# reginald-mclean/mtrl

Hardware: AMD Instinct MI355X
Metric: SAC gradient-steps/sec, MT50 width-2048 batch=128/task, 1/2/4/8 MI355X (higher is better)
Workload: dtype fp32 (2xfp16 split, per-tensor power-of-two scaled, 3 fp16 MFMA products, fp32-accurate); 1 GPU; MT50 MTMHSAC-v2 width=2048 (experiments/width_scaling/mt50_mtmhsac_v2_2048.py); num_tasks=50, width=2048, batch_per_task=128, global_batch=6400, parallelism=single, precision=split2h, exec=pipelined

## Files before the change

### include/mtsac_debug.h

```cpp
#ifndef MTSAC_DEBUG_H_
#define MTSAC_DEBUG_H_

#include <stdint.h>

#ifdef __cplusplus
extern "C" {
#endif

int mtsac_debug_gemm(int precision, int kind, int epi, int batch, int M, int N, int K, const float* A, int lda, int a_shared,
                     const float* B, int ldb, float* C, int ldc, const float* bias, const float* mask, int ldm,
                     float* db);

int mtsac_debug_gemm_bench(int precision, int kind, int epi, int batch, int M, int N, int K, int iters,
                           double* ms_per_launch);

int mtsac_debug_gemm_x3p(int epi, int M, int N, int K, const float* A, int a_kmajor, const float* B, int b_kmajor,
                         float* C, const float* bias, const float* mask, float* Csum);
int mtsac_debug_gemm_x3p_bench(int epi, int batch, int M, int N, int K, int iters, double* ms_per_launch);
int mtsac_debug_x3p_geo(int geo);

int mtsac_debug_gemm_x3f(int epi, int batch, int M, int N, int K, const float* A, const float* B, float* C,
                         const float* bias, const float* mask, float* Csum);
int mtsac_debug_gemm_x3f_ragged(int flags, int B, int N, int K, const float* A, const float* W, const float* mask,
                                const unsigned char* active, void* dense_out, void* rag_out, int* rows_out, int* info);
int mtsac_debug_gemm_fwd_bench(int which, int epi, int batch, int M, int N, int K, int iters, double* ms_per_launch);
int mtsac_debug_x3s_ti(int M, int N, int batch);
int mtsac_debug_drq_groups(int fwd, int bwd);
int mtsac_debug_drq_mfma(int mask);
int mtsac_debug_drq_legacy(int mask);
int mtsac_debug_drq_wgrad_blocks(int cap);
int mtsac_debug_drq_conv_bench(int kind, int B, int H, int W, int ci, int co, int iters, double* us_per_launch);

int mtsac_debug_drq_conv(int kind, int flags, int B, int B1, int H, int W, int ci, int co, const float* x,
                         const float* w, const float* bias, const float* w2, const float* bias2, const float* aux,
                         const float* aux2, float* out, float* out2);
int mtsac_debug_drq_conv_path(int kind, int B, int H, int W, int ci, int co, int* out);
int mtsac_debug_drq_maxpool(int B, int H, int W, int C, const float* in, float* out, unsigned char* arg,
                            const float* dout, float* din);
int mtsac_debug_drq_c51(int B, int A, int Z, int ldh, const float* hc_s, const float* hc_n, const float* hc_t,
                        const float* hb_on, const float* hb_tg, const float* rew, const float* done, const int* act,
                        float gamma_n, float vmin, float vmax, float* m, int* a_next, float* q, float* dh,
                        float* loss_b, float* logit_b);

struct mtsac_engine;
int mtsac_debug_set_pipeline(struct mtsac_engine* engine, int32_t on);

int mtsac_debug_lane_mode(struct mtsac_engine* engine);
int mtsac_debug_check_guards(struct mtsac_engine* engine);
int mtsac_debug_snapshot(struct mtsac_engine* engine, int32_t on);
int mtsac_debug_read(struct mtsac_engine* engine, int32_t id, float* dst, int64_t count);
int mtsac_debug_head_selfcheck(struct mtsac_engine* engine);
int mtsac_debug_set_bfrag(int32_t mode);
int mtsac_debug_set_actor_dense(int32_t mode);
int mtsac_debug_actor_compact(struct mtsac_engine* engine);
int mtsac_debug_bfrag(struct mtsac_engine* engine);
int mtsac_debug_force_one_stream(struct mtsac_engine* engine, int32_t on);
int mtsac_debug_set_collective_model(struct mtsac_engine* engine, int32_t nranks, double bus_gbps, int32_t flags);

struct mtsac_engine;
int mtsac_debug_timed_launch(struct mtsac_engine* engine, int32_t i, int32_t* dims, double* ms);

#ifdef __cplusplus
}
#endif
#endif
```

### mtrl_amd/_lib.py

```python

from __future__ import annotations

import ctypes
import os
import pathlib

_HERE = pathlib.Path(__file__).resolve().parent
LIB_PATH = pathlib.Path(os.environ.get("MTSAC_LIB", _HERE / "libmtsac.so"))

NUM_LOGS = 10
FP32, FP32_SPLIT3, BF16, FP32_SPLIT2H = 0, 1, 2, 3
PRECISIONS = {"fp32": FP32, "split3": FP32_SPLIT3, "bf16": BF16, "split2h": FP32_SPLIT2H}
LOG_KEYS = (
    "losses/qf_values",
    "losses/qf_loss",
    "metrics/critic_grad_magnitude",
    "metrics/critic_params_norm",
    "losses/actor_loss",
    "metrics/actor_grad_magnitude",
    "metrics/actor_params_norm",
    "metrics/explore_loss",
    "losses/alpha_loss",
    "alpha",
)
# ... 65 lines not shown
    "mtsac_last_error": (ctypes.c_char_p, []),
    "mtsac_abi_version": (ctypes.c_int, []),
    "mtsac_build_stamp": (ctypes.c_char_p, []),
    "mtsac_default_config": (None, [ctypes.POINTER(Config), I32]),
    "mtsac_create": (ctypes.c_int, [ctypes.POINTER(Config), ctypes.c_int, ctypes.POINTER(P)]),
    "mtsac_destroy": (None, [P]),
    "mtsac_param_count": (I64, [P, ctypes.c_int]),
    "mtsac_set_params": (ctypes.c_int, [P, ctypes.c_int, P, I64]),
    "mtsac_get_params": (ctypes.c_int, [P, ctypes.c_int, P, I64]),
    "mtsac_set_adam_count": (ctypes.c_int, [P, ctypes.c_int, I32]),
    "mtsac_get_adam_count": (ctypes.c_int, [P, ctypes.c_int, PI32]),
    "mtsac_buffer_add": (ctypes.c_int, [P, P, P, P, P, P]),
    "mtsac_buffer_add_stream": (ctypes.c_int, [P, P, P, P, P, P, P]),
    "mtsac_buffer_write": (ctypes.c_int, [P, I64, I64, P, P, P, P, P]),
    "mtsac_buffer_read": (ctypes.c_int, [P, I64, I64, P, P, P, P, P]),
    "mtsac_buffer_fill_synthetic": (ctypes.c_int, [P, U64]),
    "mtsac_buffer_set_state": (ctypes.c_int, [P, I64, I32]),
    "mtsac_buffer_get_state": (ctypes.c_int, [P, PI64, PI32]),
    "mtsac_buffer_set_reward_stats": (ctypes.c_int, [P, PD, PD]),
    "mtsac_buffer_get_reward_stats": (ctypes.c_int, [P, PD, PD]),
    "mtsac_rng_set": (ctypes.c_int, [P, U64, U64, U64, U64, I32, U32]),
    "mtsac_rng_get": (ctypes.c_int, [P, PU64, PU64, PU64, PU64, PI32, PU32]),
    "mtsac_sample": (ctypes.c_int, [P, P, P, P, P, P, P]),
    "mtsac_update": (ctypes.c_int, [P, ctypes.POINTER(Batch), P, P]),
    "mtsac_update_many": (ctypes.c_int, [P, I32]),
    "mtsac_get_logs": (ctypes.c_int, [P, P]),
    "mtsac_enable_graph": (ctypes.c_int, [P, I32]),
    "mtsac_synchronize": (ctypes.c_int, [P]),
    "mtsac_eval_action": (ctypes.c_int, [P, P, I32, P]),
    "mtsac_sample_action": (ctypes.c_int, [P, P, I32, P, P]),
    "mtsac_comm_unique_id_size": (ctypes.c_int, []),
    "mtsac_comm_get_unique_id": (ctypes.c_int, [P]),
    "mtsac_comm_init": (ctypes.c_int, [P, P, I32, I32]),
    "mtsac_comm_init_timeout": (ctypes.c_int, [P, P, I32, I32, ctypes.c_double]),
    "mtsac_comm_nranks": (ctypes.c_int, [P, P]),
    "mtsac_get_noise_state": (ctypes.c_int, [P, P, P]),
    "mtsac_set_noise_state": (ctypes.c_int, [P, ctypes.c_uint64, ctypes.c_uint64]),
    "mtsac_set_allreduce_hook": (ctypes.c_int, [P, ctypes.c_void_p, P]),
    "mtsac_set_collective_hook": (ctypes.c_int, [P, ctypes.c_void_p, P, ctypes.c_int32, ctypes.c_int32]),
    "mtsac_set_sharded_optimizer": (ctypes.c_int, [P, ctypes.c_int32]),
    "mtsac_memcpy": (ctypes.c_int, [P, P, I64]),
    "mtsac_set_timing": (ctypes.c_int, [P, I32]),
    "mtsac_get_timing": (ctypes.c_int, [P, I32, PD, PI32, PD]),
    "mtsac_get_timing_kernel": (ctypes.c_int, [P, I32, P, I32]),
    "mtsac_task_gradients": (ctypes.c_int, [P, ctypes.POINTER(Batch), P, P]),
    "mtsac_task_gradient_size": (I64, [P, ctypes.c_int]),
    "mtsac_get_task_gradients": (ctypes.c_int, [P, ctypes.c_int, P, I64]),
    "mtsac_set_task_gradients": (ctypes.c_int, [P, ctypes.c_int, P, I64]),
    "mtsac_task_gradient_select": (ctypes.c_int, [P, ctypes.c_int, P, P]),
    "mtsac_task_gradient_stats": (ctypes.c_int, [P, ctypes.c_int, P, ctypes.c_float, ctypes.c_float, P, P, P, P]),
    "mtsac_set_pcgrad": (ctypes.c_int, [P, I32, I32]),
    "mtsac_pcgrad_set_order": (ctypes.c_int, [P, P, P]),
    "mtsac_pcgrad_get_order": (ctypes.c_int, [P, P, P]),
    "mtsac_get_pcgrad_logs": (ctypes.c_int, [P, P]),
    "mtsac_task_gram": (ctypes.c_int, [P, ctypes.c_int, P]),
    "mtsac_task_pcgrad_solve": (ctypes.c_int, [P, ctypes.c_int, P, I32, P, P]),
    "mtsac_task_combine": (ctypes.c_int, [P, ctypes.c_int, P, P]),
    "mtsac_debug_gemm_bench": (ctypes.c_int, [ctypes.c_int] * 8 + [PD]),
    "mtsac_debug_gemm_x3p": (ctypes.c_int, [ctypes.c_int] * 4 + [P, ctypes.c_int, P, ctypes.c_int, P, P, P, P]),
    "mtsac_debug_gemm_x3p_bench": (ctypes.c_int, [ctypes.c_int] * 6 + [PD]),
    "mtsac_debug_x3p_geo": (ctypes.c_int, [ctypes.c_int]),
    "mtsac_debug_gemm_x3f": (ctypes.c_int, [ctypes.c_int] * 5 + [P] * 6),
    "mtsac_debug_gemm_x3f_ragged": (ctypes.c_int, [ctypes.c_int] * 4 + [P] * 8),
    "mtsac_debug_gemm_fwd_bench": (ctypes.c_int, [ctypes.c_int] * 7 + [PD]),
    "mtsac_debug_x3s_ti": (ctypes.c_int, [ctypes.c_int] * 3),
    "mtsac_debug_drq_groups": (ctypes.c_int, [ctypes.c_int] * 2),
    "mtsac_debug_drq_mfma": (ctypes.c_int, [ctypes.c_int]),
    "mtsac_debug_drq_legacy": (ctypes.c_int, [ctypes.c_int]),
    "mtsac_debug_drq_wgrad_blocks": (ctypes.c_int, [ctypes.c_int]),
    "mtsac_debug_drq_conv_bench": (ctypes.c_int, [ctypes.c_int] * 7 + [ctypes.POINTER(ctypes.c_double)]),
    "mtsac_debug_drq_conv": (ctypes.c_int, [ctypes.c_int] * 8 + [P] * 9),
    "mtsac_debug_drq_conv_path": (ctypes.c_int, [ctypes.c_int] * 6 + [P]),
    "mtsac_debug_drq_maxpool": (ctypes.c_int, [ctypes.c_int] * 4 + [P] * 5),
    "mtsac_debug_drq_c51": (ctypes.c_int, [ctypes.c_int] * 4 + [P] * 8 + [ctypes.c_float] * 3 + [P] * 6),
    "mtsac_debug_set_pipeline": (ctypes.c_int, [P, I32]),
    "mtsac_debug_lane_mode": (ctypes.c_int, [P]),
    "mtsac_debug_check_guards": (ctypes.c_int, [P]),
    "mtsac_debug_snapshot": (ctypes.c_int, [P, ctypes.c_int32]),
    "mtsac_debug_read": (ctypes.c_int, [P, ctypes.c_int32, P, ctypes.c_int64]),
    "mtsac_debug_head_selfcheck": (ctypes.c_int, [P]),
    "mtsac_debug_set_bfrag": (ctypes.c_int, [ctypes.c_int32]),
    "mtsac_debug_set_actor_dense": (ctypes.c_int, [ctypes.c_int32]),
    "mtsac_debug_actor_compact": (ctypes.c_int, [P]),
    "mtsac_debug_bfrag": (ctypes.c_int, [P]),
    "mtsac_debug_force_one_stream": (ctypes.c_int, [P, ctypes.c_int32]),
    "mtsac_debug_set_collective_model": (ctypes.c_int, [P, ctypes.c_int32, ctypes.c_double, ctypes.c_int32]),
    "mtsac_debug_timed_launch": (ctypes.c_int, [P, I32, PI32, PD]),
    "mtsac_debug_gemm": (
        ctypes.c_int,
        [ctypes.c_int] * 7 + [P, ctypes.c_int, ctypes.c_int, P, ctypes.c_int, P, ctypes.c_int, P, P, ctypes.c_int, P],
    ),
}


class DrqConfig(ctypes.Structure):
    _fields_ = [(n, ctypes.c_int32) for n in ("num_tasks", "n_actions", "n_atoms", "in_ch", "hw", "scale",
                                              "embed_dim", "n_hidden", "batch", "nstep")] + \
               [(n, ctypes.c_float) for n in ("gamma", "v_min", "v_max", "tau", "lr", "b1", "b2", "eps",
                                              "weight_decay", "ln_eps")] + \
               [("capacity", ctypes.c_int64), ("normalize_rewards", ctypes.c_int32), ("buffer_kind", ctypes.c_int32)]


class DrqBatch(ctypes.Structure):
    _fields_ = [(n, ctypes.c_void_p) for n in ("obs", "actions", "next_obs", "dones", "rewards", "task_ids",
                                               "crop_obs", "noise_obs", "crop_next", "noise_next")]


DRQ_PARAMS, DRQ_TARGET, DRQ_ADAM_MU, DRQ_ADAM_NU, DRQ_GRAD = 0, 1, 2, 3, 4
DRQ_NUM_LOGS = 4
DRQ_LOG_KEYS = ("losses/online_logits", "metrics/critic_grad_magnitude", "metrics/critic_params_norm",
                "losses/critic_loss")
SIGNATURES.update({
    "drq_last_error": (ctypes.c_char_p, []),
    "drq_create": (ctypes.c_int, [ctypes.POINTER(DrqConfig), ctypes.c_int, ctypes.POINTER(P)]),
    "drq_destroy": (None, [P]),
    "drq_num_params": (I64, [P]),
    "drq_set_params": (ctypes.c_int, [P, ctypes.c_int, P, I64]),
    "drq_get_params": (ctypes.c_int, [P, ctypes.c_int, P, I64]),
    "drq_set_step": (ctypes.c_int, [P, ctypes.c_int]),
    "drq_get_step": (ctypes.c_int, [P, P]),
    "drq_update": (ctypes.c_int, [P, ctypes.POINTER(DrqBatch)]),
    "drq_update_resident": (ctypes.c_int, [P, ctypes.c_int]),
    "drq_get_logs": (ctypes.c_int, [P, P]),
    "drq_q_values": (ctypes.c_int, [P, P, P, P, P, ctypes.c_int, P]),
    "drq_buffer_add": (ctypes.c_int, [P, P, P, P, P, P, P]),
    "drq_buffer_state": (ctypes.c_int, [P, PI64, PI32]),
    "drq_rng_set": (ctypes.c_int, [P, U64, U64, U64, U64, ctypes.c_int, U32]),
    "drq_sample": (ctypes.c_int, [P]),
    "drq_sample_update": (ctypes.c_int, [P, ctypes.c_int]),
    "drq_sample_rows": (ctypes.c_int, [P, P, P]),
    "drq_sample_rows_update": (ctypes.c_int, [P, P, P, ctypes.c_int]),
    "drq_rng_get": (ctypes.c_int, [P, P]),
    "drq_seed_augment": (ctypes.c_int, [P, ctypes.c_uint64]),
    "drq_task_gradient": (ctypes.c_int, [P, ctypes.POINTER(DrqBatch), ctypes.c_int, ctypes.c_int]),
    "drq_get_task_gradient": (ctypes.c_int, [P, ctypes.c_int, P, I64]),
    "drq_project_task_gradients": (ctypes.c_int, [P, ctypes.c_int, ctypes.c_int, I64, ctypes.c_int, P]),
    "drq_set_timing": (ctypes.c_int, [P, ctypes.c_int]),
    "drq_timing": (ctypes.c_int, [P, P, P, P]),
    "drq_read_batch": (ctypes.c_int, [P, P, P, P, P, P, P, P]),
    "drq_synchronize": (ctypes.c_int, [P]),
})

def source_stamp() -> str | None:
    import hashlib

    csrc = pathlib.Path(__file__).resolve().parent / "csrc"
    if not csrc.is_dir():
        return None
    rel = [f.name for pat in ("*.hip", "*.cpp", "*.h") for f in csrc.glob(pat)]
    rel += ["../../include/" + f.name for f in (csrc / ".." / ".." / "include").glob("*.h")]
    h = hashlib.sha256()
    for r in sorted(rel):
        h.update((csrc / r).read_bytes())
    return h.hexdigest()[:16]


ALLREDUCE_FN = ctypes.CFUNCTYPE(ctypes.c_int, ctypes.c_void_p, ctypes.c_void_p, ctypes.c_int64)
COLLECTIVE_FN = ctypes.CFUNCTYPE(ctypes.c_int, ctypes.c_void_p, ctypes.c_int32, ctypes.c_void_p, ctypes.c_int64)

_lib = None


def load(path: str | os.PathLike | None = None) -> ctypes.CDLL:
    global _lib
    if _lib is not None and path is None:
        return _lib
# ... 35 lines not shown
```

### mtrl_amd/csrc/debug.cpp

```cpp
#include <hip/hip_runtime.h>

#include <algorithm>
#include <cmath>
#include <cstdio>
#include <cstring>
#include <string>
#include <vector>

#include "../../include/mtsac.h"
#include "../../include/mtsac_debug.h"
#include "drq_kernels.h"
#include "kernels.h"

using namespace mtsac;

namespace {

long long up32(long long x) { return (x + 31) / 32 * 32; }

__global__ void fill_rand_f32(float* p, long long n, unsigned seed) {
  long long i = (long long)blockIdx.x * blockDim.x + threadIdx.x;
  if (i >= n) return;
  unsigned x = (unsigned)i * 2654435761u ^ seed;
  x ^= x >> 13;
// ... 434 lines not shown
  };
  std::vector<PlaneRec> hrec(5);
  std::memset(hrec.data(), 0, sizeof(PlaneRec) * hrec.size());
  const float ma = amax(Az.data(), nA), mw = amax(W, nW), mm = amax(mask, nC);
  hrec[0].e = pexp(ma); hrec[0].amax[0] = ma;
  hrec[1].e = pexp(mw); hrec[1].amax[0] = mw;
  hrec[2].e = pexp(mm); hrec[2].amax[0] = mm;
  hrec[3].e = hrec[4].e = 0x7fffffff;
  for (int i = 0; i < PLANE_REC_PARTS; ++i) hrec[3].amax[i] = hrec[4].amax[i] = 1e30f;
  PlaneRec* rec = gd.in(hrec.data(), hrec.size());
  const long long Kp = (K + 63) / 64 * 64;
  __bf16* Azp = gd.mem.get<__bf16>((size_t)3 * B * Kp * E);
  __bf16* Acp = gd.mem.get<__bf16>((size_t)3 * B * Kp * E);
  __bf16* Wp = gd.mem.get<__bf16>((size_t)3 * N * Kp * E);
  __bf16* Mp = gd.mem.get<__bf16>(3 * nC);
  const size_t out_bytes = pout ? nC * 2 * sizeof(__bf16) : nC * sizeof(float);
  unsigned char* dden = gd.out<unsigned char>(out_bytes, "dense out");
  unsigned char* drag = gd.out<unsigned char>(out_bytes, "ragged out");
  if (!gd.ok || !dAc || !rec || !Azp || !Acp || !Wp || !Mp) return -12;
  for (int z = 0; z < E; ++z) {
    SplitParams sp{};
    sp.ldx = K; sp.rows = B; sp.cols = K; sp.ldo = Kp; sp.po = (long long)B * Kp; sp.out_rows = B; sp.out_cols = (int)Kp;
    sp.e2h = &rec[0].e;
    sp.x = dAz + (size_t)z * B * K; sp.out = Azp + (size_t)z * 3 * B * Kp;
    split_planes(sp, false, 1, nullptr);
    sp.x = dAc + (size_t)z * B * K; sp.out = Acp + (size_t)z * 3 * B * Kp;
    split_planes(sp, false, 1, nullptr);
    sp.x = dW + (size_t)z * N * K; sp.rows = N; sp.out = Wp + (size_t)z * 3 * N * Kp; sp.po = (long long)N * Kp;
    sp.out_rows = N; sp.e2h = &rec[1].e; sp.frag = bfrag ? 1 : 0;
    split_planes(sp, false, 1, nullptr);
    sp.frag = 0;
    sp.x = dmask + (size_t)z * B * N; sp.ldx = N; sp.rows = B; sp.cols = N;
    sp.out = Mp + (size_t)z * 3 * B * N; sp.ldo = N; sp.po = (long long)B * N; sp.out_rows = B; sp.out_cols = N;
    sp.e2h = &rec[2].e;
    split_planes(sp, false, 1, nullptr);
  }
  SplitGemmParams g{};
  g.np = 2;
  g.lda = Kp; g.pA = (long long)B * Kp; g.sA = 3 * g.pA;
  g.B = Wp; g.ldb = Kp; g.pB = (long long)N * Kp; g.sB = 3 * g.pB;
  g.b_frag = bfrag ? 1 : 0;
  g.mask16 = Mp; g.ldm = N; g.sMask = 3ll * B * N; g.pMask = (long long)B * N;
  g.M = B; g.N = N; g.K = (int)Kp;
  g.ra = rec + 0; g.na = 1;
  g.rb = rec + 1; g.nb = 1;
  g.kmul = (float)K;
  int nparts[2] = {0, 0};
  auto outs = [&](unsigned char* o, PlaneRec* rc, int* np_) {
    g.C = nullptr; g.Cp = nullptr; g.rc = nullptr;
    if (pout) {
      g.Cp = reinterpret_cast<__bf16*>(o); g.ldcp = N; g.pC = (long long)B * N; g.sCp = 2 * g.pC;
      g.rc = rc;
    } else {
      g.C = reinterpret_cast<float*>(o); g.ldc = N; g.sC = (long long)B * N;
    }
    g.nparts = np_;
  };
  g.A = Azp;
  outs(dden, rec + 3, &nparts[0]);
  gemm_x3f(g, EPI_RELU_MASK, E, nullptr);
  if (int rc = sync_rc("dense gemm_x3f")) return rc;
  g.A = Acp;
  outs(drag, rec + 4, &nparts[1]);
  g.rag_n = d_n; g.rag_rows = d_rows; g.rag_ld = B;
  gemm_x3f_ragged(g, nullptr);
  if (int rc = sync_rc("gemm_x3f_ragged")) return rc;
  if (int rc = gd.check()) return rc;
  if (!gd.back(reinterpret_cast<unsigned char*>(dense_out), dden, out_bytes) ||
      !gd.back(reinterpret_cast<unsigned char*>(rag_out), drag, out_bytes) ||
      !gd.back(hrec.data(), rec, hrec.size()))
    return -5;
  std::copy(hrows.begin(), hrows.end(), rows_out);
  for (int k = 0; k < 2; ++k) {
    float m = 0.f;
    for (int i = 0; i < nparts[k] && i < PLANE_REC_PARTS; ++i) m = std::max(m, hrec[3 + k].amax[i]);
    info[k] = hrec[3 + k].e;
    std::memcpy(&info[2 + k], &m, sizeof(float));
  }
  info[4] = hn[0];
  info[5] = hn[1];
  return 0;
}

int mtsac_debug_gemm_fwd_bench(int which, int epi, int batch, int M, int N, int K, int iters, double* ms_per_launch) {
  const int outs = (epi >> 8) & 3;
  const int np = ((epi >> 10) & 1) ? 1 : 3;
  const bool autosplit = (epi >> 11) & 1;
  const bool fin = (epi >> 12) & 1;
  const bool h2 = (epi >> 13) & 1;
  const bool bfrag = (epi >> 14) & 1;
  epi &= 255;
  if (M < 1 || N < 1 || K < 1 || batch < 1 || iters < 1 || !ms_per_launch) return -22;
  DevBuf d;
  const long long Kp = (K + 63) / 64 * 64;
  PlaneRec* rec = d.get<PlaneRec>(3);
  if (!rec) return -12;
  float* fa = d.get<float>((size_t)M * Kp);
  float* fb = d.get<float>((size_t)N * Kp);
  float* C = d.get<float>((size_t)M * N * batch);
  float* bias = d.get<float>((size_t)N * batch);
  __bf16* Cp = d.get<__bf16>((size_t)3 * M * N * batch);
  if (!fa || !fb || !C || !bias || !Cp) return -12;
  hipLaunchKernelGGL(fill_rand_f32, dim3((unsigned)(((long long)M * Kp + 255) / 256)), dim3(256), 0, nullptr, fa,
                     (long long)M * Kp, 3u);
  hipLaunchKernelGGL(fill_rand_f32, dim3((unsigned)(((long long)N * Kp + 255) / 256)), dim3(256), 0, nullptr, fb,
                     (long long)N * Kp, 5u);
  const bool bk = which == 0;
  long long lda, pa, ldb, pb;
  plane_geom(M, (int)Kp, false, lda, pa);
  plane_geom(N, (int)Kp, bk, ldb, pb);
  __bf16* Ap = d.get<__bf16>((size_t)3 * pa * batch);
  __bf16* Bp = d.get<__bf16>((size_t)3 * pb * batch);
  if (!Ap || !Bp) return -12;
  for (int z = 0; z < batch; ++z) {
    split_into(fa, M, (int)Kp, false, Ap + 3 * pa * z, h2 ? &rec[0].e : nullptr);
    split_into(fb, N, (int)Kp, bk, Bp + 3 * pb * z, h2 ? &rec[1].e : nullptr, bfrag && !bk);
  }
  SplitGemmParams g{};
  if (h2) {
    g.ra = rec; g.rb = rec + 1; g.rc = rec + 2;
    g.kmul = (float)K;
    g.pMask = (long long)M * N;
  }
  g.A = Ap; g.lda = lda; g.pA = pa; g.sA = 3 * pa;
  g.B = Bp; g.ldb = ldb; g.pB = pb; g.sB = 3 * pb; g.b_kmajor = bk;
  g.b_frag = bfrag && !bk ? 1 : 0;
  g.C = C; g.ldc = N; g.sC = (long long)M * N;
  g.bias = bias; g.sBias = N;
  g.mask = C; g.ldm = N; g.sMask = (long long)M * N;
  g.Cp = Cp; g.ldcp = N; g.pC = (long long)M * N; g.sCp = 3 * g.pC;
  if (outs == 1) g.C = nullptr;
  if (outs == 2) g.Cp = nullptr;
  g.M = M; g.N = N; g.K = (int)Kp;
  g.splits = 1;
  g.np = h2 ? 2 : np;
  if (autosplit) {
    const long long wsf = std::max(gemm_x3f_ws_floats(M, N, (int)Kp, batch), gemm_x3p_ws_floats(M, N, (int)Kp, batch, false));
    g.ws = d.get<float>((size_t)std::max(wsf, 1LL));
    if (!g.ws) return -12;
    g.splits = -1;
    if (fin) {
      g.cnt = d.get<int>((size_t)GEMM_X3F_CNT);
      if (!g.cnt) return -12;
    }
  }
  if (which >= 1 && !gemm_x3f_ok(g, epi, batch)) return -95;
  if (which < 0 && !gemm_x3s_ok(g, epi, batch)) return -95;
  auto run = [&]() {
    if (which == -1) gemm_x3s(g, epi, batch, nullptr);
    else if (which < -1) gemm_x3s_ablate(g, -1 - which, batch, nullptr);
    else if (which >= 2) gemm_x3f_ablate(g, which - 2, batch, nullptr);
    else if (which == 1) gemm_x3f(g, epi, batch, nullptr);
    else gemm_x3p(g, epi, batch, nullptr);
  };
  run();
  hipEvent_t e0, e1;
  if (hipEventCreate(&e0) != hipSuccess || hipEventCreate(&e1) != hipSuccess) return -5;
  (void)hipEventRecord(e0, nullptr);
  for (int i = 0; i < iters; ++i) run();
  (void)hipEventRecord(e1, nullptr);
  if (hipEventSynchronize(e1) != hipSuccess) return -5;
  float ms = 0.f;
  (void)hipEventElapsedTime(&ms, e0, e1);
  *ms_per_launch = ms / iters;
  (void)hipEventDestroy(e0);
  (void)hipEventDestroy(e1);
// ... 170 lines not shown
```

### mtrl_amd/csrc/engine.cpp

```cpp
#include <hip/hip_runtime.h>
#include <rccl/rccl.h>

#include <algorithm>
#include <chrono>
#include <cmath>
#include <cstdio>
#include <cstring>
#include <mutex>
#include <string>
#include <thread>
#include <vector>

#include "../../include/mtsac.h"
#include "../../include/mtsac_debug.h"
#include "kernels.h"

using namespace mtsac;

namespace {

thread_local std::string g_last_error;
int g_bfrag_mode = -1;
int g_actor_dense_mode = -1;

int fail(int code, const std::string& msg) {
  g_last_error = msg;
  return code;
}

}
namespace mtsac {
void set_last_error(const char* msg) { g_last_error = msg; }
}
namespace {

#define HIP_TRY(expr)                                                                      \
  do {                                                                                     \
    hipError_t _e = (expr);                                                                \
    if (_e != hipSuccess)                                                                  \
      return fail(-5, std::string(#expr) + ": " + hipGetErrorString(_e));                  \
  } while (0)

constexpr int MAXD = 8;
constexpr long long ALIGN = 64;
constexpr int EXTRA = 128;
constexpr int PART = 1024;

long long align_up(long long x, long long a) { return (x + a - 1) / a * a; }

struct Net {
  int in_dim = 0, in_ld = 0, width = 0, depth = 0, T_l = 0, hd = 0, E = 1;
  long long off_hb = 0, off_hW = 0, off_b[MAXD] = {}, off_W[MAXD] = {};
  long long ms_hb = 0, ms_hW = 0, ms_b = 0, ms_W[MAXD] = {};
  long long n_flat = 0, trunk_off = 0, n_params = 0;
  std::vector<std::pair<long long, long long>> leaves;
  float *p = nullptr, *g = nullptr, *m = nullptr, *v = nullptr, *tgt = nullptr;
  float* wt[2][MAXD] = {};
  __bf16* wp[2][MAXD] = {};
  long long wld = 0, wrows = 0, arows = 0, ald = 0;
  long long krows = 0;
  bool x3f = false;
  __bf16* wtp[2][MAXD] = {};
  bool bfrag[MAXD] = {};
  float* whT = nullptr;
  float* dbp[MAXD] = {};
  int dbp_chunks[MAXD] = {};
  float* ws_wg[MAXD] = {};
  FinishSink fin_sink;
  long long wtk(int i) const { return i == 0 ? xld : ald; }
  long long wtps(int i = 1) const { return (long long)width * wtk(i); }
  long long xld = 0;
  long long aps() const { return arows * ald; }
  long long wps() const { return wrows * wld; }
  long long w0ps() const { return xld * wld; }
  long long kps(int i) const { return i == 0 ? w0ps() : wps(); }
  OptScalars* sc = nullptr;
  float *gparts = nullptr, *hparts = nullptr, *pph = nullptr, *ppt = nullptr;
  int n_pph = 0, n_ppt = 0;

  void layout(int in, int in_ld_, int W, int D, int T, int hd_, int E_) {
    in_dim = in; in_ld = in_ld_; width = W; depth = D; T_l = T; hd = hd_; E = E_;
    long long o = 0;
    auto leaf = [&](long long member, long long& off, long long& ms) {
      off = o;
      ms = member;
      leaves.push_back({o, member * E});
      n_params += member * E;
      o = align_up(o + member * E, ALIGN);
    };
    leaf((long long)T * hd, off_hb, ms_hb);
    leaf((long long)T * W * hd, off_hW, ms_hW);
    trunk_off = o;
    int fan = in;
    for (int i = 0; i < D; ++i) {
      leaf(W, off_b[i], ms_b);
      leaf((long long)fan * W, off_W[i], ms_W[i]);
      fan = W;
    }
    n_flat = o;
  }
};

}

struct mtsac_engine {
// ... 58 lines not shown
  int* task = nullptr;
  int *counts = nullptr, *rows = nullptr;
  float *u_obs = nullptr, *u_act = nullptr, *u_nobs = nullptr, *u_done = nullptr, *u_rew = nullptr;
  float *eps_n = nullptr, *eps_c = nullptr;
  float* ha[MAXD] = {};
  float* han[MAXD] = {};
  float* hc[MAXD] = {};
  float* hct[MAXD] = {};
  float* dza[MAXD] = {};
  float* dzc[MAXD] = {};
  bool planes = false;
  bool in_wgrad_planes = false;
  int np = 3;
  bool h2 = false;
  struct RecRef {
    PlaneRec* d = nullptr;
    int n = 0;
  };
  PlaneRec* recs = nullptr;
  RecRef r_in[2];
  RecRef r_w[2][2];
  RecRef r_ac[3][MAXD];
  RecRef r_dz[2][MAXD];
  RecRef r_dq, r_dout;
  float* bufmax = nullptr;
  float* ubmax = nullptr;
  float* wparts[2] = {};
  float* tparts = nullptr;
  int wgrid[2] = {}, wbh[2] = {};
  RecRef* act_rec(__bf16** actp) {
    return actp == hap || actp == hap_s2 ? r_ac[0] : actp == hcp ? r_ac[1] : actp == hctp ? r_ac[2] : nullptr;
  }
  RecRef* dz_rec(__bf16** dzp) { return dzp == dzap ? r_dz[0] : dzp == dzcp ? r_dz[1] : nullptr; }
  RecRef& w_rec(const Net& net, int which) { return r_w[&net == &critic ? 1 : 0][which]; }
  float adam_bound = 0.f;
  float adam_step_bound() const { return adam_bound; }
  static float adam_step_bound_of(double b1, double b2) {
    double r = 1.0;
    for (int t = 1; t <= 200000; t = t < 1000 ? t + 1 : t + t / 100) {
      const double f = std::sqrt(1.0 - std::pow(b2, t)) / (1.0 - std::pow(b1, t));
      r = std::max(r, f);
    }
    return (float)(1.25 * r * (1.0 - b1) / std::sqrt((1.0 - b2) * (1.0 - b1 * b1 / b2)));
  }
  void h2_gemm(SplitGemmParams& g, RecRef* a, RecRef* b, RecRef* c, float kmul, bool bias_in_b) {
    if (!h2) return;
    g.ra = a->d;
    g.na = a->n;
    g.rb = b->d;
    g.nb = b->n;
    g.rc = c ? c->d : nullptr;
    g.nparts = c ? &c->n : nullptr;
    if (c) c->n = 0;
    g.kmul = kmul;
    g.bias_in_b = bias_in_b ? 1 : 0;
  }
  __bf16* hap[MAXD] = {};
  __bf16* hap_s2[MAXD] = {};
  __bf16* hcp[MAXD] = {};
  __bf16* hctp[MAXD] = {};
  __bf16* dzap[MAXD] = {};
  __bf16* dzcp[MAXD] = {};
  float* cs_part = nullptr;
  struct InPlanes {
    const float* x;
    __bf16* p;
  };
  InPlanes inp[5] = {};
  __bf16* in_planes(const float* X) const {
    for (const InPlanes& q : inp)
      if (q.x == X) return q.p;
    if (X == xan && inp[0].p) return inp[0].p + actor.krows * actor.xld;
    return nullptr;
  }
  int split_actor_req = [] {
    const char* v = getenv("MTSAC_SPLIT_ACTOR");
    return v ? atoi(v) : -1;
  }();
  float *logpi_n = nullptr, *logpi = nullptr, *y = nullptr, *dq = nullptr, *row_a = nullptr, *row_b = nullptr,
        *row_c = nullptr, *alpha_w = nullptr, *cache = nullptr, *dout_a = nullptr;
  float* partials = nullptr;
  int *act_n = nullptr, *act_rows = nullptr, *act_slot = nullptr;
  bool actor_dense = false;
  int actor_compact_last = 0;
  float* ws_lane[5] = {};
  int* cnt_lane[5] = {};
  int* fin_cnt() {
    static const bool on = [] {
      const char* e = getenv("MTSAC_SPLITK_FIN");
      return e && atoi(e) > 0;
    }();
    return on ? cnt_lane[cur_lane] : nullptr;
  }
  int cur_lane = 0;

  bool frag_probe(const Net& net, int li) {
    static float f_;
    static __bf16 h_;
    float* F = &f_;
    __bf16* H = &h_;
    const bool is_actor = &net == &actor;
    auto base = [&](int M, long long K, long long ldb) {
      SplitGemmParams g{};
      g.np = np;
      g.lda = K;
      g.ldb = ldb;
      g.M = M;
      g.N = net.width;
      g.K = (int)K;
      g.splits = -1;
      g.ws = ws_lane[0];
      g.cnt = fin_cnt();
      g.b_frag = 1;
      return g;
    };
    std::vector<int> fwd_rows = {B};
    if (is_actor) fwd_rows.push_back((int)(net.krows + B));
    for (int M : fwd_rows)
      for (int i = li; i == li; ++i) {
        SplitGemmParams g = base(M, net.wtk(i), net.wtk(i));
        g.bias = F;
        if (i == net.depth - 1) {
          g.C = F;
          g.ldc = net.width;
        } else {
          g.Cp = H;
          g.ldcp = net.ald;
        }
        if (!gemm_x3f_ok(g, EPI_BIAS_RELU, net.E)) return false;
      }
    for (int want_db = 0; want_db < 2; ++want_db)
      for (int i = li; i == li && i > 0; ++i) {
        SplitGemmParams g = base(B, net.ald, net.wld);
        g.C = F;
        g.ldc = net.width;
        g.mask16 = H;
        g.ldm = (int)net.ald;
        if (i - 1 >= 1 || want_db) {
          g.Cp = H;
          g.ldcp = net.ald;
        }
        bool ok = false;
        if (g.Cp && want_db) {
          SplitGemmParams q = g;
          q.C = nullptr;
          q.dbp = F;
          ok = gemm_x3f_ok(q, EPI_RELU_MASK, net.E);
        } else if (g.Cp) {
          g.C = nullptr;
        }
        if (!ok && !gemm_x3f_ok(g, EPI_RELU_MASK, net.E)) return false;
      }
    return true;
  }
  float* pn = nullptr;
  float* log_alpha = nullptr;
  float *la_m = nullptr, *la_v = nullptr;
  float* alpha_tmp = nullptr;
  OptScalars* sc_alpha = nullptr;
  float* logs = nullptr;
  unsigned long long* counter = nullptr;
  int* err = nullptr;
  int roll_max = 0;
  float *r_obs = nullptr, *r_x = nullptr, *r_eps = nullptr, *r_act = nullptr, *r_lp = nullptr, *r_dummy = nullptr;
  float* r_h[MAXD] = {};
  int* r_task = nullptr;
// ... 138 lines not shown
    }();
    return g;
  }

  template <typename T>
  int alloc(T** p, size_t count, int line = __builtin_LINE()) {
    void* q = nullptr;
    size_t bytes = std::max<size_t>(count * sizeof(T), 256);
    bytes = (bytes + 255) / 256 * 256;
    const size_t G = guard_bytes();
    hipError_t e = hipMalloc(&q, bytes + 2 * G);
    if (e != hipSuccess) return fail(-12, std::string("hipMalloc failed: ") + hipGetErrorString(e));
    char* b = reinterpret_cast<char*>(q);
    e = hipMemset(b + G, 0, bytes);
    if (e == hipSuccess && G) e = hipMemset(b, 0xFF, G);
    if (e == hipSuccess && G) e = hipMemset(b + G + bytes, 0xFF, G);
    if (e != hipSuccess) return fail(-5, std::string("hipMemset failed: ") + hipGetErrorString(e));
    allocs.push_back(q);
    if (G) guards.push_back(Guard{b, bytes, line});
    *p = reinterpret_cast<T*>(b + G);
    return 0;
  }

  void dep(hipStream_t from, hipStream_t to) {
    if (from == to) return;
    if (evpool.empty()) {
      comm_error = "event pool exhausted";
      return;
    }
    hipEvent_t e = evpool[ev_next++ % evpool.size()];
    static const bool trace = getenv("MTSAC_TRACE") != nullptr;
    if (trace) fprintf(stderr, "[mtsac] dep %zu %p -> %p\n", ev_next, (void*)from, (void*)to), fflush(stderr);
    hipError_t r = hipEventRecord(e, from);
    if (trace) fprintf(stderr, "[mtsac]   record rc=%d\n", (int)r), fflush(stderr);
    if (r == hipSuccess) r = hipStreamWaitEvent(to, e, 0);
    if (trace) fprintf(stderr, "[mtsac]   wait rc=%d\n", (int)r), fflush(stderr);
    if (r != hipSuccess) comm_error = std::string("stream fork/join: ") + hipGetErrorString(r);
  }

  void t_begin(int family, double flops) {
    if (!timing) return;
    if (tl_next >= tl.size()) {
      TimedLaunch x{};
      (void)hipEventCreate(&x.a);
      (void)hipEventCreate(&x.b);
      tl.push_back(x);
    }
    tl[tl_next].family = family;
    tl[tl_next].flops = flops;
    tl[tl_next].M = tl[tl_next].N = tl[tl_next].K = tl[tl_next].batch = 0;
    (void)hipEventRecord(tl[tl_next].a, cur);
  }
  void t_end() {
    if (!timing) return;
    (void)hipEventRecord(tl[tl_next].b, cur);
    ++tl_next;
  }

  void gemm(const GemmParams& p, GemmKind kind, int epi, int batch, int family) {
    t_begin(family, 2.0 * (double)p.M * p.N * p.K * batch);
    if (timing) {
      tl[tl_next].M = p.M;
      tl[tl_next].N = p.N;
      tl[tl_next].K = p.K;
      tl[tl_next].batch = batch;
    }
    if (planes)
      gemm_x3(p, kind, epi, batch, cur);
    else
      gemm_f32(p, kind, epi, batch, cur);
    t_end();
  }

  std::string fam_kernel[8];

  void gemmp(const SplitGemmParams& p, int epi, int batch, int family) {
    t_begin(family, 2.0 * (double)p.M * p.N * p.K * batch);
    if (timing) {
      tl[tl_next].M = p.M;
      tl[tl_next].N = p.N;
      tl[tl_next].K = p.K;
      tl[tl_next].batch = batch;
    }
    if (gemm_x3f_ok(p, epi, batch)) {
      const bool split = gemm_x3f(p, epi, batch, cur) > 1;
      const bool tagged = epi == EPI_BIAS_RELU && p.tag == 1 && p.Cp && !p.C;
      fam_kernel[family] = split ? std::string("gemm_x3f_kernel<") +
                                       std::to_string(gemm_x3f_split_bm(p.M, p.N, p.K, batch)) +
                                       ", 0, true, false, false, 0, " +
                                       std::to_string(p.np == 0 ? 3 : p.np) + "> + splitk_epilogue_kernel"
                                 : std::string("gemm_x3f_kernel<") + std::to_string(gemm_x3f_bm(p, batch)) + ", " +
                                       std::to_string(epi) + ", " +
                                       (p.C ? "true" : "false") + ", " + (p.Cp ? "true" : "false") + ", " +
                                       (p.mask16 ? "true" : "false") + ", " + (tagged ? "8" : "0") + ", " +
                                       std::to_string(p.np == 0 ? 3 : p.np) + ">";
    } else if (p.b_frag) {
      comm_error = "B planes in the fragment layout and a shape gemm_x3f does not take";
    } else if (gemm_x3s_ok(p, epi, batch)) {
      gemm_x3s(p, epi, batch, cur);
      const bool tagged = epi == EPI_BIAS_RELU && p.tag == 1 && p.Cp && !p.C;
      fam_kernel[family] = std::string("gemm_x3s_kernel<") + std::to_string(gemm_x3s_ti(p.M, p.N, batch)) + ", " +
                           std::to_string(epi) + ", " + (p.C ? "true" : "false") + ", " + (p.Cp ? "true" : "false") +
                           ", " + (p.mask16 ? "true" : "false") + ", " + (tagged ? "8" : "0") + ", " +
                           std::to_string(p.np == 0 ? 3 : p.np) + ">";
    } else if ((epi == EPI_RELU_MASK && !p.mask) || (!p.C && !p.Cp)) {
      comm_error = "no plane GEMM kernel for this launch (mask16-only ReLU mask or no output)";
    } else {
      gemm_x3p(p, epi, batch, cur);
      fam_kernel[family] = "gemm_x3p_kernel";
    }
    t_end();
  }

  PlaneOut top_planes(Net& net, __bf16** dzp) {
    PlaneOut po{};
    if (planes && net.depth > 1) {
      po.p = dzp[net.depth - 1];
      po.ld = net.ald;
      po.ps = net.aps();
      po.sm = 3 * net.aps();
      if (h2) {
        RecRef& top = dz_rec(dzp)[net.depth - 1];
        RecRef& d = &net == &critic ? r_dq : r_dout;
        po.rc = top.d;
        top.n = 0;
        po.rd = d.d;
        po.nd = d.n;
        po.rw = w_rec(net, 0).d;
        po.w_add = adam_step_bound() * (&net == &critic ? cfg.critic_lr : cfg.actor_lr);
        po.kmul = (float)net.hd;
      }
    }
    return po;
  }

  void head_bwd(Net& net, const HeadParams& hp, const float* dout, long long s_dout, float** dz, __bf16** dzp,
                bool want_db, const int* slot = nullptr) {
    const int top = net.depth - 1;
    const PlaneOut po = top_planes(net, dzp);
    if (slot != nullptr) {
      head_backward_data(hp, dout, s_dout, nullptr, counts, rows, B, T_l, cur, po, nullptr, slot);
      return;
    }
    if (po.p == nullptr) {
      head_backward_data(hp, dout, s_dout, dz[top], counts, rows, B, T_l, cur, po);
      net.dbp_chunks[top] = 0;
      return;
    }
    head_backward_data(hp, dout, s_dout, nullptr, counts, rows, B, T_l, cur, po, want_db ? net.dbp[top] : nullptr);
    if (want_db) net.dbp_chunks[top] = head_backward_chunks(T_l);
  }

  bool head_bwd_both(Net& net, const HeadParams& hp, const float* dout, long long s_dout, __bf16** dzp, bool want_db) {
    const int top = net.depth - 1;
    const PlaneOut po = top_planes(net, dzp);
    if (po.p == nullptr) return false;
    float* dbp = want_db ? net.dbp[top] : nullptr;
    if (!head_backward_both(hp, dout, s_dout, nullptr, counts, rows, B, T_l, po, dbp, net.g + net.off_hW,
                            net.g + net.off_hb, cur))
      return false;
    if (want_db) net.dbp_chunks[top] = head_backward_chunks(T_l);
    return true;
  }

  void trunk_forward(Net& net, const float* params, int which, const float* X, int ldx, float** acts, __bf16** actp,
                     int M) {
    const bool pl = planes && which >= 0 && actp != nullptr;
    __bf16* xp = pl ? in_planes(X) : nullptr;
    for (int i = 0; i < net.depth; ++i) {
      const bool last = i == net.depth - 1;
      if (pl && net.x3f && (i > 0 || xp)) {
        SplitGemmParams g{};
        g.np = np;
        g.A = i == 0 ? xp : actp[i - 1];
        g.lda = i == 0 ? net.xld : net.ald;
        g.pA = i == 0 ? net.arows * net.xld : net.aps();
        g.sA = i == 0 ? 0 : 3 * net.aps();
        g.B = net.wtp[which][i];
        g.ldb = net.wtk(i);
        g.pB = net.wtps(i);
        g.sB = 3 * net.wtps(i);
        g.b_frag = net.bfrag[i] ? 1 : 0;
        if (last) {
          g.C = acts[i];
          g.ldc = net.width;
          g.sC = (long long)M * net.width;
        } else {
          g.Cp = actp[i];
          g.ldcp = net.ald;
          g.pC = net.aps();
          g.sCp = 3 * net.aps();
        }
        g.bias = params + net.off_b[i];
        g.sBias = net.ms_b;
        g.M = M;
        g.N = net.width;
        g.K = (int)net.wtk(i);
        g.tag = i == 0 ? 1 : 0;
        g.splits = -1;
        g.ws = ws_lane[cur_lane];
        g.cnt = fin_cnt();
        if (h2) {
          RecRef* ar = act_rec(actp);
          h2_gemm(g, i == 0 ? &r_in[inset_cur] : &ar[i - 1], &w_rec(net, which), last ? nullptr : &ar[i],
                  (float)(i == 0 ? net.in_dim : net.width), true);
        }
        gemmp(g, EPI_BIAS_RELU, net.E, i == 0 ? MTSAC_FAM_INPUT_FORWARD : MTSAC_FAM_FORWARD);
        continue;
      }
      if (pl && (i > 0 || xp)) {
        SplitGemmParams g{};
        g.np = np;
        g.A = i == 0 ? xp : actp[i - 1];
        g.lda = i == 0 ? net.xld : net.ald;
        g.pA = i == 0 ? net.arows * net.xld : net.aps();
        g.sA = i == 0 ? 0 : 3 * net.aps();
        g.B = net.wp[which][i];
        g.ldb = net.wld;
        g.pB = net.kps(i);
        g.sB = 3 * net.kps(i);
        g.b_kmajor = 1;
        g.C = acts[i];
        g.ldc = net.width;
        g.sC = (long long)M * net.width;
        g.bias = params + net.off_b[i];
        g.sBias = net.ms_b;
        if (!last) {
          g.Cp = actp[i];
          g.ldcp = net.ald;
          g.pC = net.aps();
          g.sCp = 3 * net.aps();
        }
        g.M = M;
        g.N = net.width;
        g.K = (int)(i == 0 ? net.xld : net.ald);
        g.tag = i == 0 ? 1 : 0;
        g.splits = -1;
        g.ws = ws_lane[cur_lane];
        g.cnt = fin_cnt();
        if (h2) {
          RecRef* ar = act_rec(actp);
          h2_gemm(g, i == 0 ? &r_in[inset_cur] : &ar[i - 1], &w_rec(net, which), last ? nullptr : &ar[i],
                  (float)(i == 0 ? net.in_dim : net.width), true);
        }
        gemmp(g, EPI_BIAS_RELU, net.E, i == 0 ? MTSAC_FAM_INPUT_FORWARD : MTSAC_FAM_FORWARD);
        continue;
      }
      GemmParams g{};
      g.A = (i == 0) ? X : acts[i - 1];
      g.lda = (i == 0) ? ldx : net.width;
      g.sA = (i == 0) ? 0 : (long long)M * net.width;
      const bool nt = !planes && which >= 0 && i > 0;
      g.B = nt ? net.wt[which][i] : params + net.off_W[i];
      g.ldb = net.width;
      g.sB = net.ms_W[i];
      g.C = acts[i];
      g.ldc = net.width;
      g.sC = (long long)M * net.width;
      g.bias = params + net.off_b[i];
      g.sBias = net.ms_b;
      g.M = M;
      g.N = net.width;
      g.K = (i == 0) ? net.in_dim : net.width;
      if (pl && !last) {
        g.Cp = actp[i];
        g.ldcp = net.ald;
        g.pC = net.aps();
        g.sCp = 3 * net.aps();
      }
      gemm(g, nt ? GEMM_NT : GEMM_NN, EPI_BIAS_RELU, net.E, i == 0 ? MTSAC_FAM_INPUT_FORWARD : MTSAC_FAM_FORWARD);
    }
  }

  bool whT_fused(const Net& net) const {
    const long long n = (long long)T_l * net.width * net.hd;
    return net.whT && net.E == 1 && net.off_hW % 4 == 0 && n % 4 == 0 && net.off_hW + n <= net.trunk_off;
  }
  void refresh_wt(Net& net, const float* params, int which, hipStream_t s, bool fused = false) {
    if (which == 0 && net.whT && net.E == 1 && !(fused && whT_fused(net)))
      head_transpose(params + net.off_hW, T_l, net.width, net.hd, net.whT, s);
    if (fused && tiles_fusable(net)) return;
    for (int i = planes ? 0 : 1; i < net.depth; ++i) {
      if (!planes) {
        transpose_f32(params + net.off_W[i], net.ms_W[i], net.wt[which][i], net.ms_W[i], net.width, net.width, net.E,
                      s);
        continue;
      }
      SplitParams sp{};
      sp.x = params + net.off_W[i];
// ... 567 lines not shown
  void reduce_rest(Net& net) {
    if (zero_of(net)) {
      const long long e = net.depth > 1 ? net.off_b[1] : net.n_flat;
      coll(1, net.g + net.trunk_off, (size_t)(e - net.trunk_off));
      return;
    }
    if (sharded() && net.depth > 1) {
      allreduce(net.g + net.trunk_off, (size_t)(net.off_b[1] - net.trunk_off));
      allreduce(net.g + net.n_flat, (size_t)EXTRA);
    } else {
      allreduce(net.g + net.trunk_off, (size_t)(net.n_flat - net.trunk_off + EXTRA));
    }
  }

  void use_inset(int k) {
    inset_cur = k;
    xa = inset[k].xa;
    xan = xa + actor.krows * ld_a;
    task = inset[k].task;
    counts = inset[k].counts;
    rows = inset[k].rows;
    inp[0].x = xa;
    inp[0].p = inset[k].xap;
  }

  void step(bool device_batch, bool device_noise, bool pipelined = false, bool join = true) {
    const int Bl = B;
    pipelined = pipelined && !build && !timing_serial;
    const bool overlap = pipelined && have_prev;
    const bool p2 = one_stream;
    if (overlap) use_inset(inset_cur ^ 1);
    counts = device_batch ? s_counts : inset[inset_cur].counts;
    rows = device_batch ? s_rows : inset[inset_cur].rows;
    if (!ev_rotate) ev_next = 0;
    segs.clear();
    actor.fin_sink.n = critic.fin_sink.n = 0;
    zstep[0] = zero_ok(actor);
    zstep[1] = zero_ok(critic);
    const float* twp = cfg.use_task_weights ? tw : nullptr;
    PolicyParams pp{};
    pp.seed = cfg.noise_seed;
    pp.counter = counter;
    pp.A = A;
    pp.ls_min = cfg.log_std_min;
    pp.ls_max = cfg.log_std_max;
    pp.ld_a_out = ld_c;
    pp.ap_ps = critic.arows * critic.xld;
    pp.ap_ld = (int)critic.xld;
    pp.counts = counts;
    pp.rows = rows;
    pp.max_rows = Bl;
    pp.T_l = T_l;
    pp.max_count = device_batch ? n : Bl;
    CriticHeadParams ch{};
    ch.rew = rew;
    ch.done = done;
    ch.log_alpha = log_alpha;
    ch.task = task;
    ch.task_begin = cfg.task_begin;
    ch.tw = twp;
    ch.gamma = cfg.gamma;
    ch.clip = cfg.clip;
    ch.T_glob = T_g;

    if (overlap) {
      hipStream_t w = p2 ? s2 : st;
      (void)hipStreamWaitEvent(w, ev_ap[step_par ^ 1], 0);
      if (cfg.use_task_weights) (void)hipStreamWaitEvent(w, ev_tail[step_par ^ 1], 0);
    }
    pf_issue = overlap && p2;
    const int s_in = seg({}, 0, [&] {
      GatherParams gp = gather_params();
      if (device_batch) {
        replay_indices(rng, jump, buf_size, n, idx, cur);
        replay_gather(gp, cur);
      } else {
        if (h2) user_batch_max(gp, Bl);
        batch_scatter(gp, u_obs, u_act, u_nobs, u_done, u_rew, Bl, cur);
        task_rows(task, Bl, T_l, counts, rows, Bl, cur);
      }
      if (cfg.use_task_weights) row_alpha(task, cfg.task_begin, log_alpha, T_g, Bl, 1, row_c, tw, cur);
    });
    const bool ol = overlap || lanes_alt;
    const int s_cf = seg({s_in}, ol ? 2 : 1, [&] { trunk_forward(critic, critic.p, 0, xc, ld_c, hc, hcp, Bl); });
    pf_issue = false;
    if (overlap && !p2) (void)hipStreamWaitEvent(st, ev_tail[step_par ^ 1], 0);
    const bool split_af = split_actor_req > 0 || (split_actor_req < 0 && dev_collective() && one_stream && !build &&
                                                  !timing_serial && !lanes_alt && Bl <= 2048);
    auto pi_s = [&](PolicyParams& q) {
      q = pp;
      q.head = head(actor, actor.p, ha[actor.depth - 1], Bl, task);
      q.eps = device_noise ? nullptr : eps_c;
      q.stream_id = 2;
      q.a_out = xcp;
      q.a_planes = in_planes(xcp);
      q.ap_rec = h2 ? r_in[inset_cur].d : nullptr;
      q.logpi = logpi;
      q.cache = cache;
    };
    const int s_af = seg({s_in}, ol ? 0 : 2, [&] {
      if (split_af) {
        trunk_forward(actor, actor.p, 0, xan, ld_a, han, hap_s2, Bl);
        PolicyParams qn = pp;
        qn.head = head(actor, actor.p, han[actor.depth - 1], Bl, task);
        qn.eps = device_noise ? nullptr : eps_n;
        qn.stream_id = 1;
        qn.a_out = xcn;
        qn.a_planes = in_planes(xcn);
        qn.ap_rec = h2 ? r_in[inset_cur].d : nullptr;
        qn.logpi = logpi_n;
        policy_head(qn, cur);
        return;
      }
      trunk_forward(actor, actor.p, 0, xa, ld_a, ha, hap, Ma);
      PolicyParams q = pp;
      q.head = head(actor, actor.p, ha[actor.depth - 1], Bl, task);
      q.eps = device_noise ? nullptr : eps_c;
      q.stream_id = 2;
      q.a_out = xcp;
      q.a_planes = in_planes(xcp);
      q.ap_rec = h2 ? r_in[inset_cur].d : nullptr;
      q.logpi = logpi;
      q.cache = cache;
      PolicyParams qn = pp;
      qn.head = head(actor, actor.p, han[actor.depth - 1], Bl, task);
      qn.eps = device_noise ? nullptr : eps_n;
      qn.stream_id = 1;
      qn.a_out = xcn;
      qn.a_planes = in_planes(xcn);
      qn.ap_rec = q.ap_rec;
      qn.logpi = logpi_n;
      policy_head_pair(q, qn, cur);
      if (snap_on)
        (void)hipMemcpyAsync(dbg_snap[0], ha[actor.depth - 1], sizeof(float) * Ma * actor.width,
                             hipMemcpyDeviceToDevice, cur);
    });
    const bool fuse_td = one_stream || timing_serial;
    const int s_tg = seg({s_af}, 0, [&] {
      trunk_forward(critic, critic.tgt, 1, xcn, ld_c, hct, hctp, Bl);
      if (!fuse_td) {
        CriticHeadParams c = ch;
        c.head = head(critic, critic.tgt, hct[critic.depth - 1], Bl, task);
        c.mode = CH_TARGET;
        c.logpi = logpi_n;
        c.y_out = y;
        critic_head(c, cur);
      }
    });
    const HeadParams chp = head(critic, critic.p, hc[critic.depth - 1], Bl, task);
    bool c_both = false;
    const int s_cl = seg({s_cf, s_tg}, 1, [&] {
      CriticHeadParams c = ch;
      c.head = chp;
      c.mode = CH_CRITIC;
      c.y = y;
      if (fuse_td) {
        c.fused_target = 1;
        c.thead = head(critic, critic.tgt, hct[critic.depth - 1], Bl, task);
        c.logpi = logpi_n;
        c.y_out = y;
      }
      c.dq = dq;
      c.row_a = row_a;
      c.row_b = row_b;
      c.inv_norm = 1.0f / ((float)critic.E * (float)B_glob);
      if (h2) {
        c.dq_rec = r_dq.d;
        c.dq_parts = &r_dq.n;
      }
      critic_head(c, cur);
      c_both = head_bwd_both(critic, chp, dq, Bl, dzcp, true);
      if (!c_both) head_bwd(critic, chp, dq, Bl, dzc, dzcp, true);
      if (sharded()) {
        const float* ins[2] = {row_a, row_b};
        reduce_rows(ins, 2, Bl, critic.g + critic.n_flat + 1, cur);
      }
    });
    const int s_chw = seg({s_cl}, 3, [&] {
      if (!c_both)
        head_backward_weight(chp, dq, Bl, counts, rows, Bl, critic.g + critic.off_hW, critic.g + critic.off_hb, cur);
    });
    int s_afs = s_af;
    const int s_cb = backward_segs(critic, critic.p, xc, ld_c, hc, hcp, dzc, dzcp, s_cl, s_chw, Bl, [&] {
      if (split_af)
        s_afs = seg({s_in}, 1, [&] {
          trunk_forward(actor, actor.p, 0, xa, ld_a, ha, hap, Bl);
          PolicyParams q;
          pi_s(q);
          policy_head(q, cur);
        });
    });
    const int s_co = seg({s_cb}, 1, [&] {
      if (sharded()) head_sq(critic);
      reduce_rest(critic);
      optimize(critic, cfg.critic_lr, cfg.critic_max_grad_norm, true, 0);
      refresh_wt(critic, critic.p, 0, cur, true);
      refresh_wt(critic, critic.tgt, 1, cur, true);
    });
    const int s_ap = seg({s_co, s_af, s_afs}, 1, [&] {
      trunk_forward(critic, critic.p, 0, xcp, ld_c, hc, hcp, Bl);
      CriticHeadParams c = ch;
      c.head = head(critic, critic.p, hc[critic.depth - 1], Bl, task);
      c.mode = CH_ACTOR;
      c.logpi = logpi;
      c.dq = dq;
      c.row_a = row_c;
      c.alpha_w = alpha_w;
      c.inv_norm = 1.0f / (float)B_glob;
      if (h2) {
        c.dq_rec = r_dq.d;
        c.dq_parts = &r_dq.n;
      }
      critic_head(c, cur);
      const bool rag = actor_compact(Bl);
      actor_compact_last = rag ? 1 : 0;
      if (rag) active_rows(dq, critic.E, Bl, act_n, act_rows, act_slot, cur);
      head_bwd(critic, c.head, dq, Bl, dzc, dzcp, false, rag ? act_slot : nullptr);
      for (int i = critic.depth - 1; i > 0; --i)
        dgrad_layer(critic, critic.p, hc, hcp, dzc, dzcp, i, Bl, false, rag ? 1 : 0);
      ActionGradParams ag{};
      ag.dz1 = dzc[0];
      ag.slot = rag ? act_slot : nullptr;
      ag.W0 = critic.p + critic.off_W[0];
      ag.s_dz = (long long)Bl * critic.width;
      ag.s_W0 = critic.ms_W[0];
      ag.E = critic.E;
      ag.B = Bl;
      ag.Wc = critic.width;
      ag.A = A;
      ag.cache = cache;
      ag.alpha_w = alpha_w;
      ag.ls_min = cfg.log_std_min;
      ag.ls_max = cfg.log_std_max;
      ag.dout = dout_a;
      if (h2) {
        ag.dout_rec = r_dout.d;
        ag.dout_parts = &r_dout.n;
      }
      action_grad(ag, cur);
      if (snap_on)
        (void)hipMemcpyAsync(dbg_snap[1], ha[actor.depth - 1], sizeof(float) * Ma * actor.width,
                             hipMemcpyDeviceToDevice, cur);
      if (sharded()) {
        const float* ins[1] = {row_c};
        reduce_rows(ins, 1, Bl, actor.g + actor.n_flat + 1, cur);
      }
    });
    if (pipelined) (void)hipEventRecord(ev_ap[step_par], segs[s_ap].lane);
    const HeadParams ahp = head(actor, actor.p, ha[actor.depth - 1], Bl, task);
    const bool a_both = top_planes(actor, dzap).p != nullptr && actor.width % 4 == 0;
    const int s_ahw = seg({s_ap}, 3, [&] {
      if (!a_both)
        head_backward_weight(ahp, dout_a, 0, counts, rows, Bl, actor.g + actor.off_hW, actor.g + actor.off_hb, cur);
    });
    const int s_ad = seg({s_ap}, 1, [&] {
      if (!(a_both && head_bwd_both(actor, ahp, dout_a, 0, dzap, true))) head_bwd(actor, ahp, dout_a, 0, dza, dzap, true);
    });
    const int s_ab = backward_segs(actor, actor.p, xa, ld_a, ha, hap, dza, dzap, s_ad, s_ahw, Bl);
    const int s_tail = seg({s_ab}, 1, [&] {
      AlphaParams al = alpha_params();
      if (sharded()) alpha_grad(al, cur);
      if (sharded()) head_sq(actor);
      reduce_rest(actor);
      optimize(actor, cfg.actor_lr, cfg.actor_max_grad_norm, false, 1);
      refresh_wt(actor, actor.p, 0, cur, true);
      allreduce(pn + 2, 2);
      StepFinish f = finish_params(al);
      step_finish(f, cur);
    });
    if (pipelined) (void)hipEventRecord(ev_tail[step_par], segs[s_tail].lane);
    if (!build && (join || !pipelined)) {
      for (const Seg& s : segs)
        if (s.lane != st && s.ev) (void)hipStreamWaitEvent(st, s.ev, 0);
    }
    have_prev = pipelined && !join;
    step_par ^= 1;
    cur = st;
  }

  float* tg[2] = {};
  long long tgP[2] = {};
  unsigned* sel_prefix = nullptr;
  long long* sel_rank = nullptr;
  unsigned* sel_hist = nullptr;
  double *ps_gram_part = nullptr, *ps_l1_part = nullptr, *ps_gram = nullptr, *ps_l1 = nullptr;
  unsigned long long *ps_counts = nullptr, *ps_nz = nullptr;
  float* ps_thr = nullptr;
  static constexpr int PS_GRID = 512;

  static std::vector<long long> dense_offsets(const Net& net) {
    std::vector<long long> off;
    long long o = 0;
    for (const auto& lf : net.leaves) {
      off.push_back(o);
      o += lf.second;
    }
    off.push_back(o);
    return off;
// ... 680 lines not shown
  if ((rc = e->alloc(&e->store, (size_t)c.capacity * e->T_l * e->R))) return bad(rc);
  if ((rc = e->alloc(&e->buf_size, 1))) return bad(rc);
  if ((rc = e->alloc(&e->rng, 1))) return bad(rc);
  if ((rc = e->alloc(&e->jump, 65 * 4))) return bad(rc);
  if ((rc = e->alloc(&e->idx, e->n))) return bad(rc);
  if ((rc = e->alloc(&e->rmin, e->T_l))) return bad(rc);
  if ((rc = e->alloc(&e->rmax, e->T_l))) return bad(rc);
  e->Ma = (int)(e->actor.krows + B);
  for (auto& q : e->inset) {
    if ((rc = e->alloc(&q.xa, (size_t)e->Ma * e->ld_a))) return bad(rc);
    if ((rc = e->alloc(&q.task, B)) || (rc = e->alloc(&q.counts, e->T_l)) || (rc = e->alloc(&q.rows, (size_t)e->T_l * B)))
      return bad(rc);
  }
  e->xa = e->inset[0].xa;
  e->xan = e->xa + e->actor.krows * e->ld_a;
  e->task = e->inset[0].task;
  e->counts = e->inset[0].counts;
  e->rows = e->inset[0].rows;
  {
    std::vector<int> sc(e->T_l, e->n), sr((size_t)e->T_l * B, 0);
    for (int t = 0; t < e->T_l; ++t)
      for (int i = 0; i < e->n; ++i) sr[(size_t)t * B + i] = i * e->T_l + t;
    if ((rc = e->alloc(&e->s_counts, e->T_l)) || (rc = e->alloc(&e->s_rows, (size_t)e->T_l * B))) return bad(rc);
    if (hipMemcpy(e->s_counts, sc.data(), sizeof(int) * sc.size(), hipMemcpyHostToDevice) != hipSuccess ||
        hipMemcpy(e->s_rows, sr.data(), sizeof(int) * sr.size(), hipMemcpyHostToDevice) != hipSuccess)
      return bad(fail(-5, "row lists"));
  }
  if ((rc = e->alloc(&e->xc, (size_t)B * e->ld_c))) return bad(rc);
  if ((rc = e->alloc(&e->xcn, (size_t)B * e->ld_c))) return bad(rc);
  if ((rc = e->alloc(&e->xcp, (size_t)B * e->ld_c))) return bad(rc);
  for (float** p : {&e->rew, &e->done, &e->tw, &e->logpi_n, &e->logpi, &e->y, &e->row_a, &e->row_b, &e->row_c,
                    &e->alpha_w, &e->u_done, &e->u_rew})
    if ((rc = e->alloc(p, B))) return bad(rc);

  if ((rc = e->alloc(&e->u_obs, (size_t)B * e->D))) return bad(rc);
  if ((rc = e->alloc(&e->u_nobs, (size_t)B * e->D))) return bad(rc);
  if ((rc = e->alloc(&e->u_act, (size_t)B * e->A))) return bad(rc);
  if ((rc = e->alloc(&e->eps_n, (size_t)B * e->A))) return bad(rc);
  if ((rc = e->alloc(&e->eps_c, (size_t)B * e->A))) return bad(rc);
  for (int i = 0; i < c.actor_depth; ++i) {
    if ((rc = e->alloc(&e->ha[i], (size_t)e->Ma * c.actor_width))) return bad(rc);
    e->han[i] = e->ha[i] + e->actor.krows * c.actor_width;
    if ((rc = e->alloc(&e->dza[i], (size_t)B * c.actor_width))) return bad(rc);
  }
  for (int i = 0; i < c.critic_depth; ++i)
    for (float** p : {&e->hc[i], &e->hct[i], &e->dzc[i]})
      if ((rc = e->alloc(p, (size_t)c.num_critics * B * c.critic_width))) return bad(rc);
  if (e->planes) {
    for (Net* net : {&e->actor, &e->critic}) {
      const bool cr = net == &e->critic;
      const size_t np = (size_t)net->E * 3 * net->aps();
      for (int i = 0; i + 1 < net->depth; ++i) {
        if ((rc = e->alloc(cr ? &e->hcp[i] : &e->hap[i], np))) return bad(rc);
        if (!cr) e->hap_s2[i] = e->hap[i] + net->krows * net->ald;
        if (cr && (rc = e->alloc(&e->hctp[i], np))) return bad(rc);
      }
      const int d0 = e->in_wgrad_planes ? 0 : 1;
      for (int i = d0; i < net->depth; ++i)
        if ((rc = e->alloc(cr ? &e->dzcp[i] : &e->dzap[i], np))) return bad(rc);
      const long long chunks = std::max<long long>({(long long)COLSUM_CHUNKS, gemm_x3f_max_row_tiles(e->B),
                                                    head_backward_chunks(e->T_l)});
      for (int i = d0; i < net->depth; ++i)
        if ((rc = e->alloc(&net->dbp[i], (size_t)(net->E * chunks * net->width)))) return bad(rc);
    }
    {
      const float* xs[5] = {e->xa, e->xan, e->xc, e->xcn, e->xcp};
      for (int k = 0; k < 5; ++k) {
        const Net& net = k < 2 ? e->actor : e->critic;
        if (k == 1) continue;
        e->inp[k].x = xs[k];
        if ((rc = e->alloc(&e->inp[k].p, (size_t)3 * net.arows * net.xld))) return bad(rc);
      }
      e->inset[0].xap = e->inp[0].p;
      if ((rc = e->alloc(&e->inset[1].xap, (size_t)3 * e->actor.arows * e->actor.xld))) return bad(rc);
    }
    const int wmax = std::max(c.actor_width, c.critic_width);
    if ((rc = e->alloc(&e->cs_part, (size_t)std::max(1, c.num_critics) * COLSUM_CHUNKS * wmax))) return bad(rc);
  }
  if ((rc = e->alloc(&e->dq, (size_t)c.num_critics * B))) return bad(rc);
  if ((rc = e->alloc(&e->act_n, (size_t)std::max(2, c.num_critics)))) return bad(rc);
  if ((rc = e->alloc(&e->act_rows, (size_t)c.num_critics * B))) return bad(rc);
  if ((rc = e->alloc(&e->act_slot, (size_t)c.num_critics * B))) return bad(rc);
  {
    const char* v = getenv("MTSAC_ACTOR_DENSE");
    e->actor_dense = g_actor_dense_mode >= 0 ? g_actor_dense_mode != 0 : (v && atoi(v) != 0);
  }
  if ((rc = e->alloc(&e->cache, (size_t)B * 5 * e->A))) return bad(rc);
  if ((rc = e->alloc(&e->dout_a, (size_t)B * 2 * e->A))) return bad(rc);
  if ((rc = e->alloc(&e->partials, 2 * PART))) return bad(rc);
  if ((rc = e->alloc(&e->zparts, 256)) || (rc = e->alloc(&e->zscr, 2048))) return bad(rc);
  if ((rc = e->alloc(&e->pn, 4))) return bad(rc);
  if ((rc = e->alloc(&e->log_alpha, e->T_g))) return bad(rc);
  if ((rc = e->alloc(&e->la_m, e->T_g))) return bad(rc);
  if ((rc = e->alloc(&e->la_v, e->T_g))) return bad(rc);
  if ((rc = e->alloc(&e->alpha_tmp, e->T_g))) return bad(rc);
  if ((rc = e->alloc(&e->sc_alpha, 1))) return bad(rc);
  if ((rc = e->alloc(&e->logs, MTSAC_NUM_LOGS))) return bad(rc);
  if ((rc = e->alloc(&e->counter, 1))) return bad(rc);
  if ((rc = e->alloc(&e->err, 2))) return bad(rc);
  const int rm = e->roll_max;
  if ((rc = e->alloc(&e->r_obs, (size_t)rm * e->D))) return bad(rc);
  if ((rc = e->alloc(&e->r_x, (size_t)rm * e->ld_a))) return bad(rc);
  if ((rc = e->alloc(&e->r_eps, (size_t)rm * e->A))) return bad(rc);
  if ((rc = e->alloc(&e->r_act, (size_t)rm * e->A))) return bad(rc);
  if ((rc = e->alloc(&e->r_lp, rm))) return bad(rc);
  if ((rc = e->alloc(&e->r_dummy, (size_t)rm * (e->ld_c + 4)))) return bad(rc);
  if ((rc = e->alloc(&e->r_task, rm))) return bad(rc);
  for (int i = 0; i < c.actor_depth; ++i)
    if ((rc = e->alloc(&e->r_h[i], (size_t)rm * c.actor_width))) return bad(rc);

  unsigned long long jt[65 * 4];
  pcg_jump_table(jt);
  if (hipMemcpy(e->jump, jt, sizeof(jt), hipMemcpyHostToDevice) != hipSuccess) return bad(fail(-5, "jump table"));
  std::vector<float> la(e->T_g, std::log(c.initial_temperature));
  if (hipMemcpy(e->log_alpha, la.data(), sizeof(float) * e->T_g, hipMemcpyHostToDevice) != hipSuccess)
    return bad(fail(-5, "log_alpha"));
  {
    std::vector<double> mn(e->T_l, INFINITY), mx(e->T_l, -INFINITY);
    if (c.normalize_rewards == 2) {
      std::fill(mn.begin(), mn.end(), 0.0);
      std::fill(mx.begin(), mx.end(), 1.0);
    }
    if (hipMemcpy(e->rmin, mn.data(), sizeof(double) * e->T_l, hipMemcpyHostToDevice) != hipSuccess ||
        hipMemcpy(e->rmax, mx.data(), sizeof(double) * e->T_l, hipMemcpyHostToDevice) != hipSuccess)
      return bad(fail(-5, "reward stats"));
  }
  if (hipHostMalloc((void**)&e->stage_h, sizeof(float) * mtsac_engine::NSTAGE * e->T_l * e->R) != hipSuccess)
    return bad(fail(-12, "pinned staging"));
  for (hipEvent_t& x : e->stage_ev)
    if (hipEventCreateWithFlags(&x, hipEventDisableTiming) != hipSuccess) return bad(fail(-5, "event"));
  if (hipEventCreateWithFlags(&e->add_ev, hipEventDisableTiming) != hipSuccess) return bad(fail(-5, "event"));
  for (int k = 0; k < mtsac_engine::NSTAGE; ++k)
    if (hipEventCreateWithFlags(&e->dstage_ev[k], hipEventDisableTiming) != hipSuccess ||
        hipEventCreateWithFlags(&e->dpack_ev[k], hipEventDisableTiming) != hipSuccess)
      return bad(fail(-5, "event"));
  if ((rc = e->alloc(&e->dstage, (size_t)mtsac_engine::NSTAGE * e->T_l * e->R))) return bad(rc);
  for (int k = 0; k < 2; ++k)
    if (hipEventCreateWithFlags(&e->ev_ap[k], hipEventDisableTiming) != hipSuccess ||
        hipEventCreateWithFlags(&e->ev_tail[k], hipEventDisableTiming) != hipSuccess)
      return bad(fail(-5, "event"));
  if (hipDeviceSynchronize() != hipSuccess) return bad(fail(-5, "device synchronize"));
  *out = e;
  return 0;
}

void mtsac_destroy(mtsac_engine* h) { delete h; }

static Net* net_of(mtsac_engine* h, int which, float** buf) {
  switch (which) {
    case MTSAC_ACTOR: *buf = h->actor.p; return &h->actor;
    case MTSAC_CRITIC: *buf = h->critic.p; return &h->critic;
    case MTSAC_CRITIC_TARGET: *buf = h->critic.tgt; return &h->critic;
    case MTSAC_ACTOR_ADAM_MU: *buf = h->actor.m; return &h->actor;
    case MTSAC_ACTOR_ADAM_NU: *buf = h->actor.v; return &h->actor;
    case MTSAC_CRITIC_ADAM_MU: *buf = h->critic.m; return &h->critic;
    case MTSAC_CRITIC_ADAM_NU: *buf = h->critic.v; return &h->critic;
    default: return nullptr;
  }
}

static float* alpha_buf(mtsac_engine* h, int which) {
  switch (which) {
    case MTSAC_LOG_ALPHA_PARAMS: return h->log_alpha;
    case MTSAC_ALPHA_ADAM_MU: return h->la_m;
    case MTSAC_ALPHA_ADAM_NU: return h->la_v;
    default: return nullptr;
  }
}
// ... 831 lines not shown
  h->timing_serial = enable == 2;
  return 0;
}
int mtsac_get_timing(mtsac_engine* h, int32_t family, double* total_ms, int32_t* launches, double* flops) {
  if (!h || !total_ms || !launches || !flops) return fail(-22, "null argument");
  HIP_TRY(hipStreamSynchronize(h->st));
  double ms = 0.0, fl = 0.0;
  int nl = 0;
  for (size_t i = 0; i < h->tl_next && i < h->tl.size(); ++i) {
    if (h->tl[i].family != family) continue;
    float t = 0.f;
    HIP_TRY(hipEventElapsedTime(&t, h->tl[i].a, h->tl[i].b));
    ms += t;
    fl += h->tl[i].flops;
    ++nl;
  }
  *total_ms = ms;
  *launches = nl;
  *flops = fl;
  return 0;
}

int mtsac_get_timing_kernel(mtsac_engine* h, int32_t family, char* buf, int32_t n) {
  if (!h || !buf || n < 1) return fail(-22, "null argument");
  if (family < 0 || family >= 8) return fail(-22, "unknown family");
  std::snprintf(buf, (size_t)n, "%s", h->fam_kernel[family].c_str());
  return 0;
}

int mtsac_debug_set_pipeline(mtsac_engine* h, int32_t on) {
  if (!h) return fail(-22, "null engine");
  const int was = h->pipeline_req;
  h->pipeline_req = on < 0 ? -1 : on != 0 ? 1 : 0;
  return was;
}

int mtsac_debug_set_collective_model(mtsac_engine* h, int32_t nranks, double bus_gbps, int32_t flags) {
  if (!h) return fail(-22, "null engine");
  if (h->comm || h->hook || h->chook) return fail(-16, "a communicator or collective hook is installed");
  if (nranks < 1 || (nranks > 1 && !(bus_gbps > 0.0))) return fail(-22, "nranks >= 1 and bus_gbps > 0");
  HIP_TRY(hipStreamSynchronize(h->st));
  h->cmodel.nranks = nranks;
  h->cmodel.gbps = bus_gbps;
  h->cmodel.poison = (flags & 1) != 0;
  h->cmodel.blocks = ((flags >> 8) & 255) ? (flags >> 8) & 255 : 8;
  if (h->cmodel.poison) {
    long long need = 0;
    for (const Net* net : {&h->actor, &h->critic}) need = std::max(need, net->n_flat - net->trunk_off + EXTRA);
    if (need > h->cm_cap) {
      int rc = h->alloc(&h->cm_shadow, (size_t)need);
      if (rc) return rc;
      h->cm_cap = need;
    }
  }
  if (h->gexec) {
    (void)hipGraphExecDestroy(h->gexec);
    (void)hipGraphDestroy(h->graph);
    h->gexec = nullptr;
    h->graph = nullptr;
  }
  return 0;
}

int mtsac_debug_force_one_stream(mtsac_engine* h, int32_t on) {
  if (!h) return fail(-22, "null engine");
  HIP_TRY(hipStreamSynchronize(h->st));
  mtsac_engine::Registry& r = mtsac_engine::registry();
  std::lock_guard<std::mutex> g(r.mu);
  h->force_one = on != 0;
  mtsac_engine::relane(r);
  return 0;
}

int mtsac_debug_set_bfrag(int32_t mode) {
  if (mode < -1 || mode > 1) return fail(-22, "bfrag mode is -1, 0 or 1");
  g_bfrag_mode = mode;
  return 0;
}

int mtsac_debug_set_actor_dense(int32_t mode) {
  if (mode < -1 || mode > 1) return fail(-22, "actor dense mode is -1, 0 or 1");
  g_actor_dense_mode = mode;
  return 0;
}

int mtsac_debug_actor_compact(mtsac_engine* h) {
  if (!h) return fail(-22, "null engine");
  return h->actor_compact_last;
}

int mtsac_debug_bfrag(mtsac_engine* h) {
  if (!h) return fail(-22, "null engine");
  int m = 0;
  for (int i = 0; i < MAXD && i < 8; ++i) m |= (h->actor.bfrag[i] ? 1 << i : 0) | (h->critic.bfrag[i] ? 256 << i : 0);
  return m;
}

int mtsac_debug_check_guards(mtsac_engine* h) {
  if (!h) return fail(-22, "null engine");
  const size_t G = mtsac_engine::guard_bytes();
  if (G == 0) return fail(-95, "guard zones are off (set MTSAC_GUARD_BYTES before the engine is created)");
  HIP_TRY(hipDeviceSynchronize());
  std::vector<unsigned char> buf(G);
  int bad = 0;
  std::string msg;
  for (const auto& g : h->guards)
    for (int side = 0; side < 2; ++side) {
      HIP_TRY(hipMemcpy(buf.data(), g.base + (side ? G + g.bytes : 0), G, hipMemcpyDeviceToHost));
      size_t first = G, n = 0;
      for (size_t i = 0; i < G; ++i)
        if (buf[i] != 0xFF) {
          if (first == G) first = i;
          ++n;
        }
      if (n) {
        ++bad;
        if (bad <= 8)
          msg += "alloc@line " + std::to_string(g.line) + " (" + std::to_string(g.bytes) + " B) " +
                 (side ? "back" : "front") + " guard: " + std::to_string(n) + " bytes written, first at " +
                 (side ? "+" : "-") + std::to_string(side ? first : G - first) + "; ";
      }
    }
  if (bad) g_last_error = msg;
  return bad;
}

int mtsac_debug_snapshot(mtsac_engine* h, int32_t on) {
  if (!h) return fail(-22, "null engine");
  if (on && !h->dbg_snap[0])
    for (float*& q : h->dbg_snap)
      if (int rc = h->alloc(&q, (size_t)h->Ma * h->actor.width)) return rc;
  h->snap_on = on != 0;
  return 0;
}

int mtsac_debug_head_selfcheck(mtsac_engine* h) {
  if (!h) return fail(-22, "null engine");
  if (h->actor.hd != 8 || h->actor.width % 4 != 0 || h->counts == nullptr) return fail(-95, "needs hd 8, W % 4 == 0 and a step");
  if (!h->dbg_hw)
    if (int rc = h->alloc(&h->dbg_hw, (size_t)h->T_l * h->actor.width * 8 + (size_t)h->T_l * 8)) return rc;
  const HeadParams ahp = h->head(h->actor, h->actor.p, h->ha[h->actor.depth - 1], h->B, h->task);
  head_backward_weight_inject(ahp, h->dout_a, 0, h->counts, h->rows, h->B, h->T_l, h->dbg_hw,
                              h->dbg_hw + (size_t)h->T_l * h->actor.width * 8, h->st);
  HIP_TRY(hipGetLastError());
  return 0;
}

int mtsac_debug_read(mtsac_engine* h, int32_t id, float* dst, int64_t count) {
  if (!h || !dst) return fail(-22, "null argument");
  const float* src = nullptr;
  int64_t n = 0;
  switch (id) {
    case 0: src = h->ha[h->actor.depth - 1]; n = (int64_t)h->Ma * h->actor.width; break;
    case 1: src = h->dbg_snap[0]; n = (int64_t)h->Ma * h->actor.width; break;
    case 2: src = h->dbg_snap[1]; n = (int64_t)h->Ma * h->actor.width; break;
    case 3: src = h->dout_a; n = (int64_t)h->B * 2 * h->A; break;
    case 4: src = h->actor.g; n = h->actor.trunk_off; break;
    default: return fail(-22, "unknown buffer id");
  }
  if (!src) return fail(-22, "buffer not allocated (mtsac_debug_snapshot)");
  if (count != n) return fail(-22, "count must be " + std::to_string(n));
  HIP_TRY(hipStreamSynchronize(h->st));
  HIP_TRY(hipMemcpy(dst, src, sizeof(float) * n, hipMemcpyDeviceToHost));
  return 0;
}

// ... 138 lines not shown
```

### mtrl_amd/csrc/gemm_x3f.hip

```cpp
#include <algorithm>
#include <cstdlib>

#include "gemm_x3f_impl.h"

namespace mtsac {
namespace x3fk {

constexpr int BM0 = 208;

constexpr int BF16_BM[] = {48, 80, 208, 400};

static int bf16_bm(int M, int N, int batch) {
  const long long ny = (N + 255) / 256;
  int best = BM0;
  double best_t = 1e30;
  for (int bm : BF16_BM) {
    const long long rounds = ((M + bm - 1) / bm * ny * batch + 255) / 256;
    const double t = (double)rounds * std::max(8.0 * bm, 4.57 * (bm + 256));
    if (t < best_t - 1e-9) {
      best_t = t;
      best = bm;
    }
  }
  return best;
// ... 107 lines not shown
        best_cost = cost;
        best = {bm, sp};
      }
    }
  }
  return best;
}
}

int gemm_x3f_splits(int M, int N, int K, int batch) { return x3fk::split_plan(M, N, K, batch).s; }

static int x3f_slices(const SplitGemmParams& p, int epi, int batch);
int splitk_dbp_rows();
static bool x3f_fin_ok(const SplitGemmParams& p, int epi, int batch);
int gemm_x3f_out_bm(const SplitGemmParams& p, int epi, int batch) {
  if (x3f_slices(p, epi, batch) <= 1) return gemm_x3f_bm(p, batch);
  return x3f_fin_ok(p, epi, batch) ? x3fk::split_plan(p.M, p.N, p.K, batch).bm : splitk_dbp_rows();
}
int gemm_x3f_split_bm(int M, int N, int K, int batch) { return x3fk::split_plan(M, N, K, batch).bm; }

long long gemm_x3f_ws_floats(int M, int N, int K, int batch) {
  const int s = gemm_x3f_splits(M, N, K, batch);
  return s > 1 ? (long long)batch * s * M * N : 0;
}

int gemm_x3f_tiles(int M, int N, int batch) {
  return ((M + x3fk::BM0 - 1) / x3fk::BM0) * ((N + x3fk::BN - 1) / x3fk::BN) * batch;
}

bool gemm_x3f_fin_supported(const SplitGemmParams& q, int epi, int bm);
bool gemm_x3f_fin(const SplitGemmParams& q, int epi, int bm, dim3 grid, hipStream_t st);

static bool x3f_fin_ok(const SplitGemmParams& p, int epi, int batch) {
  if (p.cnt == nullptr) return false;
  const x3fk::SplitPlan sp = x3fk::split_plan(p.M, p.N, p.K, batch);
  if (p.np == 2 && sp.s != 2) return false;
  const long long tiles = (long long)((p.M + sp.bm - 1) / sp.bm) * ((p.N + x3fk::BN - 1) / x3fk::BN) * batch;
  return tiles <= GEMM_X3F_CNT && gemm_x3f_fin_supported(p, epi, sp.bm);
}

static int x3f_slices(const SplitGemmParams& p, int epi, int batch) {
  if (p.splits >= 0 || p.ws == nullptr) return 1;
  if (p.dbp != nullptr && !x3f_fin_ok(p, epi, batch) && !(epi == EPI_BIAS_RELU || (epi == EPI_RELU_MASK && p.mask16)))
    return 1;
  static const bool bf16_split = [] {
    const char* e = getenv("MTSAC_BF16_SPLIT");
    return e && atoi(e) != 0;
  }();
  if (p.np == 1 && !bf16_split && x3fk::bf16_workgroups(p.M, p.N, batch) >= 128) return 1;
  if (epi == EPI_RELU_MASK && !p.mask16 && !p.mask) return 1;
  if (p.N % 4 != 0 || (p.C && p.ldc % 4 != 0) || (p.Cp && p.ldcp % 4 != 0)) return 1;
  return gemm_x3f_splits(p.M, p.N, p.K, batch);
}

static long long x3f_workgroups(const SplitGemmParams& p, int epi, int batch) {
  const int S = x3f_slices(p, epi, batch);
  if (S == 1) return p.np == 1 ? x3fk::bf16_workgroups(p.M, p.N, batch) : gemm_x3f_tiles(p.M, p.N, batch);
  const int bm = x3fk::split_plan(p.M, p.N, p.K, batch).bm;
  return (long long)((p.M + bm - 1) / bm) * ((p.N + x3fk::BN - 1) / x3fk::BN) * batch * S;
}

bool gemm_x3f_ok(const SplitGemmParams& p, int epi, int batch) {
  return !p.a_kmajor && !p.b_kmajor && p.K % x3fk::KS == 0 && p.N % 8 == 0 && p.lda % 8 == 0 && p.ldb % 8 == 0 &&
         (!p.C || p.ldc % 4 == 0) && (!p.Cp || p.ldcp % 8 == 0) && (epi != EPI_RELU_MASK || p.ldm % 8 == 0) &&
         (epi != EPI_STORE) && x3f_workgroups(p, epi, batch) >= 192 &&
         (p.C || p.Cp) && (long long)p.N * p.ldb * 2 < (1ll << 31) &&
         (!p.b_frag || (p.N % 16 == 0 && p.ldb % 32 == 0));
}

bool gemm_x3f_ragged_ok(const SplitGemmParams& p, int epi, int batch) {
  return p.np == 2 && batch == 2 && epi == EPI_RELU_MASK && p.mask16 != nullptr && p.dbp == nullptr &&
         (p.C != nullptr) != (p.Cp != nullptr) && x3fk::g_x3f_order == 0 && gemm_x3f_ok(p, epi, batch) &&
         x3f_slices(p, epi, batch) == 1;
}

void gemm_x3f_ragged(const SplitGemmParams& p, hipStream_t st) {
  using namespace x3fk;
  const dim3 grid((unsigned)(((p.M + BM0 - 1) / BM0) * ((p.N + BN - 1) / BN) * 2));
  if (p.nparts) *p.nparts = (int)grid.x;
  if (p.Cp != nullptr)
    hipLaunchKernelGGL((gemm_x3f_kernel<BM0, EPI_RELU_MASK, false, true, true, TAG_RAGGED, 2>), grid, dim3(512), 0, st, p);
  else
    hipLaunchKernelGGL((gemm_x3f_kernel<BM0, EPI_RELU_MASK, true, false, true, TAG_RAGGED, 2>), grid, dim3(512), 0, st, p);
}

int gemm_x3f(const SplitGemmParams& p0, int epi, int batch, hipStream_t st) {
  using namespace x3fk;
  const int S = x3f_slices(p0, epi, batch);
  if (S > 1 && x3f_fin_ok(p0, epi, batch)) {
    SplitGemmParams q = p0;
    q.kchunk = (p0.K / KS + S - 1) / S * KS;
    q.splits = (p0.K + q.kchunk - 1) / q.kchunk;
    const int bm = split_plan(p0.M, p0.N, p0.K, batch).bm;
    const unsigned tiles = (unsigned)(((p0.M + bm - 1) / bm) * ((p0.N + BN - 1) / BN) * batch);
    const dim3 grid(tiles * (unsigned)q.splits);
    if (q.splits > 1 && (q.np != 2 || q.splits == 2) && gemm_x3f_fin(q, epi, bm, grid, st)) {
      if (p0.nparts) *p0.nparts = (int)tiles;
      return q.splits;
    }
  }
  if (S > 1) {
    SplitGemmParams q = p0;
    q.splits = S;
    q.kchunk = (p0.K / KS + S - 1) / S * KS;
    q.C = p0.ws;
    q.ldc = p0.N;
    q.sC = (long long)S * p0.M * p0.N;
    q.Cp = nullptr;
    q.dbp = nullptr;
    const int S_eff = (p0.K + q.kchunk - 1) / q.kchunk;
    q.splits = S_eff;
    const int bm = split_plan(p0.M, p0.N, p0.K, batch).bm;
    const dim3 grid((unsigned)(((p0.M + bm - 1) / bm) * ((p0.N + BN - 1) / BN) * batch * S_eff));
    const dim3 blk(512);
    switch (bm * 4 + (p0.np == 1 ? 1 : p0.np == 2 ? 2 : 3)) {
      case BMS * 4 + 2: hipLaunchKernelGGL((gemm_x3f_kernel<BMS, EPI_STORE, true, false, false, 0, 2>), grid, blk, 0, st, q); break;
      case BM0 * 4 + 2: hipLaunchKernelGGL((gemm_x3f_kernel<BM0, EPI_STORE, true, false, false, 0, 2>), grid, blk, 0, st, q); break;
      case BMT * 4 + 2: hipLaunchKernelGGL((gemm_x3f_kernel<BMT, EPI_STORE, true, false, false, 0, 2>), grid, blk, 0, st, q); break;
      case BMS * 4 + 1: hipLaunchKernelGGL((gemm_x3f_kernel<BMS, EPI_STORE, true, false, false, 0, 1>), grid, blk, 0, st, q); break;
      case BMS * 4 + 3: hipLaunchKernelGGL((gemm_x3f_kernel<BMS, EPI_STORE, true, false, false, 0, 3>), grid, blk, 0, st, q); break;
      case BMT * 4 + 1: hipLaunchKernelGGL((gemm_x3f_kernel<BMT, EPI_STORE, true, false, false, 0, 1>), grid, blk, 0, st, q); break;
      case BMT * 4 + 3: hipLaunchKernelGGL((gemm_x3f_kernel<BMT, EPI_STORE, true, false, false, 0, 3>), grid, blk, 0, st, q); break;
      case BM0 * 4 + 1: hipLaunchKernelGGL((gemm_x3f_kernel<BM0, EPI_STORE, true, false, false, 0, 1>), grid, blk, 0, st, q); break;
      default: hipLaunchKernelGGL((gemm_x3f_kernel<BM0, EPI_STORE, true, false, false, 0, 3>), grid, blk, 0, st, q); break;
    }
    SplitGemmParams f = p0;
    f.sC = p0.sC;
    splitk_finish(f, epi, S_eff, batch, st);
    return S_eff;
  }
  const SplitGemmParams& p = p0;
  const int bm = gemm_x3f_bm(p, batch);
  const dim3 grid((unsigned)(((p.M + bm - 1) / bm) * ((p.N + BN - 1) / BN) * batch));
  if (p.nparts) *p.nparts = (int)grid.x;
  const bool c = p.C != nullptr, pl = p.Cp != nullptr, m16 = p.mask16 != nullptr;
  if (epi == EPI_BIAS_RELU && p.tag == 1 && pl && !c) {
    launch<EPI_BIAS_RELU, false, true, false, TAG_INPUT>(p, grid, st, bm);
  } else if (epi == EPI_BIAS_RELU) {
    if (c && pl) launch<EPI_BIAS_RELU, true, true, false>(p, grid, st, bm);
    else if (c) launch<EPI_BIAS_RELU, true, false, false>(p, grid, st, bm);
    else launch<EPI_BIAS_RELU, false, true, false>(p, grid, st, bm);
  } else {
    if (m16) {
      if (c && pl) launch<EPI_RELU_MASK, true, true, true>(p, grid, st, bm);
      else if (c) launch<EPI_RELU_MASK, true, false, true>(p, grid, st, bm);
      else launch<EPI_RELU_MASK, false, true, true>(p, grid, st, bm);
    } else {
      if (c && pl) launch<EPI_RELU_MASK, true, true, false>(p, grid, st, bm);
      else if (c) launch<EPI_RELU_MASK, true, false, false>(p, grid, st, bm);
      else launch<EPI_RELU_MASK, false, true, false>(p, grid, st, bm);
    }
  }
  return 1;
}

}
```

### mtrl_amd/csrc/gemm_x3f_impl.h

```cpp
#pragma once
#include <type_traits>

#include "gemm_x3p_impl.h"

#ifndef X3F_DEEP_B
#define X3F_DEEP_B 1
#endif
#ifndef X3F_EPI_GROUP
#define X3F_EPI_GROUP 2
#endif

namespace mtsac {
namespace x3fk {

using x3pk::glds16;
typedef float f32x4 __attribute__((ext_vector_type(4)));
typedef unsigned u32x4 __attribute__((ext_vector_type(4)));

constexpr int BN = 256;
constexpr int TAG_INPUT = 8;
constexpr int TAG_RAGGED = 16;
constexpr int KS = 64;

__device__ inline bf16x8 gload_frag(const __bf16* base, unsigned voff) {
  bf16x8 r;
  asm volatile("global_load_dwordx4 %0, %1, %2" : "=v"(r) : "v"(voff), "s"(base) : "memory");
  return r;
}

template <int N, int NP, int JB>
__device__ inline void wait_vm(bf16x8 (&b)[JB][NP]) {
  if constexpr (JB == 2 && NP == 3)
    asm volatile("s_waitcnt vmcnt(%6)"
                 : "+v"(b[0][0]), "+v"(b[0][1]), "+v"(b[0][2]), "+v"(b[1][0]), "+v"(b[1][1]), "+v"(b[1][2])
                 : "n"(N)
                 : "memory");
  else if constexpr (JB == 2 && NP == 2)
    asm volatile("s_waitcnt vmcnt(%4)"
                 : "+v"(b[0][0]), "+v"(b[0][1]), "+v"(b[1][0]), "+v"(b[1][1])
                 : "n"(N)
                 : "memory");
  else if constexpr (NP == 2)
    asm volatile("s_waitcnt vmcnt(%8)"
                 : "+v"(b[0][0]), "+v"(b[0][1]), "+v"(b[1][0]), "+v"(b[1][1]), "+v"(b[2][0]), "+v"(b[2][1]),
                   "+v"(b[3][0]), "+v"(b[3][1])
                 : "n"(N)
                 : "memory");
  else if constexpr (JB == 2)
    asm volatile("s_waitcnt vmcnt(%2)" : "+v"(b[0][0]), "+v"(b[1][0]) : "n"(N) : "memory");
  else if constexpr (NP == 3)
    asm volatile("s_waitcnt vmcnt(%12)"
                 : "+v"(b[0][0]), "+v"(b[0][1]), "+v"(b[0][2]), "+v"(b[1][0]), "+v"(b[1][1]), "+v"(b[1][2]),
                   "+v"(b[2][0]), "+v"(b[2][1]), "+v"(b[2][2]), "+v"(b[3][0]), "+v"(b[3][1]), "+v"(b[3][2])
                 : "n"(N)
                 : "memory");
  else
    asm volatile("s_waitcnt vmcnt(%4)" : "+v"(b[0][0]), "+v"(b[1][0]), "+v"(b[2][0]), "+v"(b[3][0]) : "n"(N) : "memory");
}

template <int BM, int EPI, bool C_OUT, bool P_OUT, bool MASK16, int ABL = 0, int NP = 3, int WV = 8, bool FIN = false>
__global__ __launch_bounds__(64 * WV, 1) void gemm_x3f_kernel(SplitGemmParams p) {
  constexpr int JB = BN / 16 / WV;
  constexpr int TI = BM / 16;
  constexpr int PLANE = BM * 128;
  constexpr int STAGE = NP * PLANE;
  constexpr int NJ = NP * BM / 8;
  constexpr int PMAX = (NJ + WV - 1) / WV;
  constexpr int P0 = (ABL & 512) ? (PMAX + 1) / 2 : PMAX;
  constexpr int PW = (ABL & 512) ? P0 : PMAX - 1;
  constexpr int EG = (!FIN && NP >= 2) ? X3F_EPI_GROUP : 1;
  constexpr int EPI_LDS = (2 * EG * 16 * (BN + 4) + WV * BN + 16) * 4;
  constexpr bool DEEP = NP == 1 && BM <= 208 && ABL == 0 && EPI != EPI_STORE && !FIN && X3F_DEEP_B;
  constexpr int SMEM0 = 2 * STAGE > EPI_LDS ? 2 * STAGE : EPI_LDS;
  constexpr int SMEM = SMEM0 + (FIN ? 16 : 0);
  static_assert(BM % 16 == 0 && SMEM <= 160 * 1024, "tile");
  static_assert(PMAX - 1 >= PW || NJ % WV == 0, "every wave issues >= PW pieces in the first half step");
  static_assert(JB * 16 * WV == BN && (JB == 2 || JB == 4), "column slabs");
  __shared__ __attribute__((aligned(16))) char smem[SMEM];
  const unsigned lds_base = (unsigned)(unsigned long long)(x3pk::lds_void*)smem;

  const int t = threadIdx.x, lane = t & 63;
  const int wave = __builtin_amdgcn_readfirstlane(t >> 6);
  __builtin_assume(wave >= 0 && wave < WV);
  const int mine = (wave < NJ % WV || NJ % WV == 0) ? PMAX : PMAX - 1;

  constexpr bool RAG = ABL == TAG_RAGGED;
  static_assert(!RAG || (NP == 2 && !FIN && EPI == EPI_RELU_MASK && MASK16), "ragged: the split2h data grad only");
  const int ny = (p.N + BN - 1) / BN, nx = (p.M + BM - 1) / BM;
  int lin = blockIdx.x;
  int rag_t0 = 0, rag_n0 = 0, rag_n1 = 0;
  if constexpr (RAG) {
    rag_n0 = min(max(p.rag_n[0], 0), p.M);
    rag_n1 = min(max(p.rag_n[1], 0), p.M);
    rag_t0 = (rag_n0 + BM - 1) / BM;
    const int n = min((rag_t0 + (rag_n1 + BM - 1) / BM) * ny, (int)gridDim.x);
    if (lin >= n) {
      if (P_OUT && t == 0 && lin < PLANE_REC_PARTS) p.rc->amax[lin] = 0.f;
      return;
    }
    const int q8 = n / 8, r8 = n % 8, x = lin % 8;
    lin = (x < r8 ? x * (q8 + 1) : r8 * (q8 + 1) + (x - r8) * q8) + lin / 8;
  } else {
    const int n = gridDim.x, q8 = n / 8, r8 = n % 8, x = lin % 8;
    lin = (x < r8 ? x * (q8 + 1) : r8 * (q8 + 1) + (x - r8) * q8) + lin / 8;
  }
  const int nsplit = p.splits > 1 ? p.splits : 1;
  const int tiles = ny * nx * (int)(gridDim.x / nsplit / (ny * nx));
  const int sl = RAG ? 0 : FIN ? lin % nsplit : lin / tiles;
  lin = RAG ? lin : FIN ? lin / nsplit : lin - sl * tiles;
  const int tile_id = lin;
  const int by = RAG ? lin % ny : p.order ? (lin / nx) % ny : lin % ny;
  const int bx = RAG ? lin / ny - (lin / ny >= rag_t0 ? rag_t0 : 0) : p.order ? lin % nx : (lin / ny) % nx;
  const int z = RAG ? (lin / ny >= rag_t0 ? 1 : 0) : lin / (ny * nx);
  const int Mz = RAG ? (z ? rag_n1 : rag_n0) : p.M;
  const int m0 = bx * BM, n0 = by * BN;
  const int k0 = nsplit > 1 ? sl * p.kchunk : 0;
  const __bf16* __restrict__ A = p.A + z * p.sA + k0;
  const int bks = p.b_frag ? 16 : 1;
  const __bf16* B = p.B + z * p.sB + (long long)bks * k0;
  const int nk = (nsplit > 1 ? min(p.kchunk, p.K - k0) : p.K) / KS;

  auto piece = [&](int j, int k0, unsigned st) {
    const int q = j / (BM / 8), rg = j % (BM / 8);
    int row = m0 + 8 * rg + (lane >> 3);
    const int pc = lane & 7;
    const int c = pc ^ (row & 7);
    row = row < Mz ? row : Mz - 1;
    glds16(A + q * p.pA + (long long)row * p.lda + k0 + 8 * c, st + q * PLANE + rg * 1024);
  };
  auto wave_piece = [&](int qi, int k0, unsigned st) {
    const int j = wave + WV * qi;
    if (j < NJ) piece(j, k0, st);
  };
  auto afrag = [&](const char* cur, int i, int s, int q) {
    const int r = 16 * i + (lane & 15);
    const int c = 4 * s + (lane >> 4);
    return *reinterpret_cast<const bf16x8*>(cur + q * PLANE + r * 128 + 16 * (c ^ (r & 7)));
  };

  unsigned boff[JB];
#pragma unroll
  for (int j = 0; j < JB; ++j) {
    int n = n0 + 16 * JB * wave + 16 * j + (lane & 15);
    n = n < p.N ? n : p.N - 1;
    boff[j] = (unsigned)(((long long)n * p.ldb + 8 * (lane >> 4)) * 2);
    if (p.b_frag) {
      int nb = (n0 + 16 * JB * wave + 16 * j) >> 4;
      nb = nb < (p.N >> 4) ? nb : (p.N >> 4) - 1;
      boff[j] = (unsigned)(((long long)nb * (p.ldb >> 5) * 512 + 8 * lane) * 2);
    }
    if (ABL & 64) boff[j] = (unsigned)((long long)(n0 + 16 * JB * wave + 16 * j) * p.ldb * 2 + 16 * lane);
  }
  auto bload = [&](bf16x8 (&b)[JB][NP], int k) {
#pragma unroll
    for (int q = 0; q < NP; ++q) {
      const __bf16* base = B + q * p.pB + bks * k;
#pragma unroll
      for (int j = 0; j < JB; ++j) b[j][q] = gload_frag(base, boff[j]);
    }
  };

  f32x4 acc[TI][JB];
#pragma unroll
  for (int i = 0; i < TI; ++i)
#pragma unroll
    for (int j = 0; j < JB; ++j) acc[i][j] = f32x4{0.f, 0.f, 0.f, 0.f};

  bf16x8 b0[JB][NP], b1[JB][NP];
  if ((ABL & 4) && wave >= 4) __builtin_amdgcn_s_setprio(1);
#pragma unroll
// ... 143 lines not shown
  float omx = 0.f;
  const int oc = 8 * (lane & 31);
  const int col = n0 + oc;
  const bool colok = col < p.N;
  const long long slab = (long long)p.M * p.N;
  const float* ws_z = FIN ? p.ws + (long long)z * nsplit * slab : nullptr;
  const bool pair = FIN && nsplit == 2;
  auto write_slab = [&](bool scale) {
    const __amdgpu_buffer_rsrc_t slab_rs = __builtin_amdgcn_make_buffer_rsrc(
        (void*)(p.ws + ((long long)z * nsplit + sl) * slab), (short)0, -1, 0x00020000);
#pragma unroll
    for (int i = 0; i < TI; ++i) {
      float* tb = img + (i & 1) * 16 * TS;
#pragma unroll
      for (int j = 0; j < JB; ++j)
#pragma unroll
        for (int r = 0; r < 4; ++r) tb[(4 * (lane >> 4) + r) * TS + 16 * JB * wave + 16 * j + (lane & 15)] = acc[i][j][r];
      __syncthreads();
#pragma unroll
      for (int rp = 0; rp < RP; ++rp) {
        const int orow = 2 * (wave + WV * rp) + (lane >> 5);
        const int row = m0 + 16 * i + orow;
        if (row >= p.M || !colok) continue;
        float4 u = *reinterpret_cast<const float4*>(tb + orow * TS + oc);
        float4 v = *reinterpret_cast<const float4*>(tb + orow * TS + oc + 4);
        if (scale) {
          u.x *= unscale; u.y *= unscale; u.z *= unscale; u.w *= unscale;
          v.x *= unscale; v.y *= unscale; v.z *= unscale; v.w *= unscale;
        }
        const unsigned o = (unsigned)(((long long)row * p.N + col) * 4);
        __builtin_amdgcn_raw_buffer_store_b128(__builtin_bit_cast(u32x4, u), slab_rs, (int)o, 0, 16);
        __builtin_amdgcn_raw_buffer_store_b128(__builtin_bit_cast(u32x4, v), slab_rs, (int)o + 16, 0, 16);
      }
    }
    asm volatile("s_waitcnt vmcnt(0)" ::: "memory");
    __syncthreads();
  };
  if constexpr (FIN) {
    int* last = reinterpret_cast<int*>(smem + SMEM0);
    if (pair) {
      if (t == 0) *last = __hip_atomic_fetch_add(p.cnt + tile_id, 1, __ATOMIC_RELAXED, __HIP_MEMORY_SCOPE_AGENT);
      __syncthreads();
      const int tk = *last;
      if (tk == 0) {
        write_slab(NP == 2);
        if (t == 0) {
          asm volatile("s_waitcnt vmcnt(0)" ::: "memory");
          __hip_atomic_fetch_add(p.cnt + tile_id, 2, __ATOMIC_RELAXED, __HIP_MEMORY_SCOPE_AGENT);
        }
        return;
      }
      if (t == 0) {
        if (tk == 1)
          while (__hip_atomic_load(p.cnt + tile_id, __ATOMIC_RELAXED, __HIP_MEMORY_SCOPE_AGENT) != 4)
            __builtin_amdgcn_s_sleep(2);
        __hip_atomic_store(p.cnt + tile_id, 0, __ATOMIC_RELAXED, __HIP_MEMORY_SCOPE_AGENT);
      }
      __syncthreads();
    } else {
      write_slab(NP == 2);
      if (t == 0) {
        const int tk = __hip_atomic_fetch_add(p.cnt + tile_id, 1, __ATOMIC_RELAXED, __HIP_MEMORY_SCOPE_AGENT);
        const int me = tk == nsplit - 1;
        if (me) __hip_atomic_store(p.cnt + tile_id, 0, __ATOMIC_RELAXED, __HIP_MEMORY_SCOPE_AGENT);
        *last = me;
      }
      __syncthreads();
      if (*last == 0) return;
      if (t == 0) {
        __builtin_amdgcn_fence(__ATOMIC_ACQUIRE, "agent");
        asm volatile("s_waitcnt vmcnt(0)" ::: "memory");
      }
      __syncthreads();
    }
  }
  if constexpr (NP == 2) {
    if (P_OUT) {
      const int ec = gemm_out_exp(p, mscr);
      oscale = exp2i(ec);
      if ((FIN ? tile_id : (int)blockIdx.x) == 0 && t == 0) p.rc->e = ec;
    }
  }
  float bias[8];
  if (EPI == EPI_BIAS_RELU && colok) {
    const float4 u = *reinterpret_cast<const float4*>(p.bias + z * p.sBias + col);
    const float4 v = *reinterpret_cast<const float4*>(p.bias + z * p.sBias + col + 4);
    bias[0] = u.x; bias[1] = u.y; bias[2] = u.z; bias[3] = u.w;
    bias[4] = v.x; bias[5] = v.y; bias[6] = v.z; bias[7] = v.w;
  }
  float* C = C_OUT ? p.C + z * p.sC + (FIN ? 0ll : (long long)sl * p.M * p.ldc) : nullptr;
  __bf16* Cp = P_OUT ? p.Cp + z * p.sCp : nullptr;
  float csum[8] = {0.f, 0.f, 0.f, 0.f, 0.f, 0.f, 0.f, 0.f};
  constexpr int PB = !FIN ? 1 : TI < 8 ? TI : 8;
  float pre[PB][8];
  static_assert(!FIN || RP == 1, "the in-launch finish runs with 8 waves (one row pair per wave and block)");
  const bool two = pair;
  const __amdgpu_buffer_rsrc_t other_rs =
      __builtin_amdgcn_make_buffer_rsrc((void*)(ws_z + (1 - sl) * slab), (short)0, -1, 0x00020000);
  auto prefetch = [&](int i0) {
#pragma unroll
    for (int ii = 0; ii < PB; ++ii) {
      const int row = m0 + 16 * (i0 + ii) + 2 * wave + (lane >> 5);
      if (i0 + ii < TI && row < p.M && colok) {
        const int o = (int)(((long long)row * p.N + col) * 4);
        const float4 a0 = __builtin_bit_cast(float4, __builtin_amdgcn_raw_buffer_load_b128(other_rs, o, 0, 16));
        const float4 a1 = __builtin_bit_cast(float4, __builtin_amdgcn_raw_buffer_load_b128(other_rs, o + 16, 0, 16));
        pre[ii][0] = a0.x; pre[ii][1] = a0.y; pre[ii][2] = a0.z; pre[ii][3] = a0.w;
        pre[ii][4] = a1.x; pre[ii][5] = a1.y; pre[ii][6] = a1.z; pre[ii][7] = a1.w;
      }
    }
  };
  if (two) prefetch(0);
  constexpr bool MPF = EPI == EPI_RELU_MASK && MASK16 && NP == 2 && !FIN;
  constexpr int MG = MPF ? EG * RP : 1;
  i16x8 mbuf[2][MG][2];
  auto mask_load = [&](int i0, int b) {
#pragma unroll
    for (int g = 0; g < EG; ++g)
#pragma unroll
      for (int rp = 0; rp < RP; ++rp) {
        int row = m0 + 16 * (i0 + g) + 2 * (wave + WV * rp) + (lane >> 5);
        row = row < Mz ? row : Mz - 1;
        if constexpr (RAG) row = p.rag_rows[z * p.rag_ld + row];
        const __bf16* mp = p.mask16 + z * p.sMask + (long long)row * p.ldm + (colok ? col : 0);
        mbuf[b][g * RP + rp][0] = __builtin_bit_cast(i16x8, *reinterpret_cast<const bf16x8*>(mp));
        mbuf[b][g * RP + rp][1] = __builtin_bit_cast(i16x8, *reinterpret_cast<const bf16x8*>(mp + p.pMask));
      }
  };
  if constexpr (MPF) mask_load(0, 0);
#pragma unroll
  for (int i0 = 0; i0 < TI; i0 += EG) {
    float* tb0 = img + ((i0 / EG) & 1) * EG * 16 * TS;
    if constexpr (MPF) {
      if (i0 + EG < TI) mask_load(i0 + EG, ((i0 / EG) + 1) & 1);
    }
#pragma unroll
    for (int g = 0; g < EG; ++g) {
      if (i0 + g >= TI) break;
#pragma unroll
      for (int j = 0; j < JB; ++j)
#pragma unroll
        for (int r = 0; r < 4; ++r)
          tb0[(16 * g + 4 * (lane >> 4) + r) * TS + 16 * JB * wave + 16 * j + (lane & 15)] = acc[i0 + g][j][r];
    }
    __syncthreads();
#pragma unroll
    for (int g = 0; g < EG; ++g) {
    const int i = i0 + g;
    if (i >= TI) break;
    if (two && i > 0 && i % PB == 0) prefetch(i);
    float* tb = tb0 + g * 16 * TS;
#pragma unroll
    for (int rp = 0; rp < RP; ++rp) {
    const int orow = 2 * (wave + WV * rp) + (lane >> 5);
    const float4 u = *reinterpret_cast<const float4*>(tb + orow * TS + oc);
    const float4 v = *reinterpret_cast<const float4*>(tb + orow * TS + oc + 4);
    const int row = m0 + 16 * i + orow;
    if (row >= Mz || !colok) continue;
    if ((ABL & 128) && p.M > 0) continue;
    float e[8] = {u.x, u.y, u.z, u.w, v.x, v.y, v.z, v.w};
    if constexpr (NP == 2) {
#pragma unroll
      for (int c = 0; c < 8; ++c) e[c] *= unscale;
    }
    if (two) {
#pragma unroll
      for (int c = 0; c < 8; ++c) e[c] = e[c] + pre[i % PB][c];
    } else if constexpr (FIN) {
      float o[8];
#pragma unroll
      for (int c = 0; c < 8; ++c) o[c] = e[c];
      const float* w = ws_z + (long long)row * p.N + col;
      for (int s = 0; s < nsplit; ++s) {
        float x[8];
        if (s == sl) {
#pragma unroll
          for (int c = 0; c < 8; ++c) x[c] = o[c];
        } else {
          const float4 a0 = *reinterpret_cast<const float4*>(w + s * slab);
          const float4 a1 = *reinterpret_cast<const float4*>(w + s * slab + 4);
          x[0] = a0.x; x[1] = a0.y; x[2] = a0.z; x[3] = a0.w;
          x[4] = a1.x; x[5] = a1.y; x[6] = a1.z; x[7] = a1.w;
        }
#pragma unroll
        for (int c = 0; c < 8; ++c) e[c] = s == 0 ? x[c] : e[c] + x[c];
      }
    }
    if (EPI == EPI_BIAS_RELU) {
#pragma unroll
      for (int c = 0; c < 8; ++c) e[c] = fmaxf(e[c] + bias[c], 0.f);
    }
    if (EPI == EPI_RELU_MASK) {
      if (MPF) {
        const i16x8& mh = mbuf[(i0 / EG) & 1][g * RP + rp][0];
        const i16x8& ml = mbuf[(i0 / EG) & 1][g * RP + rp][1];
#pragma unroll
        for (int c = 0; c < 8; ++c) e[c] = (mh[c] > 0 || ml[c] > 0) ? e[c] : 0.f;
      } else if (MASK16 && NP == 2) {
        const __bf16* mp = p.mask16 + z * p.sMask + (long long)row * p.ldm + col;
        const i16x8 mh = __builtin_bit_cast(i16x8, *reinterpret_cast<const bf16x8*>(mp));
        const i16x8 ml = __builtin_bit_cast(i16x8, *reinterpret_cast<const bf16x8*>(mp + p.pMask));
#pragma unroll
        for (int c = 0; c < 8; ++c) e[c] = (mh[c] > 0 || ml[c] > 0) ? e[c] : 0.f;
      } else if (MASK16) {
        const bf16x8 mk = *reinterpret_cast<const bf16x8*>(p.mask16 + z * p.sMask + (long long)row * p.ldm + col);
#pragma unroll
        for (int c = 0; c < 8; ++c) e[c] = (float)mk[c] > 0.f ? e[c] : 0.f;
      } else {
        const float* mp = p.mask + z * p.sMask + (long long)row * p.ldm + col;
        const float4 a0 = *reinterpret_cast<const float4*>(mp), a1 = *reinterpret_cast<const float4*>(mp + 4);
        const float mk[8] = {a0.x, a0.y, a0.z, a0.w, a1.x, a1.y, a1.z, a1.w};
#pragma unroll
        for (int c = 0; c < 8; ++c) e[c] = mk[c] > 0.f ? e[c] : 0.f;
      }
    }
#pragma unroll
    for (int c = 0; c < 8; ++c) csum[c] += e[c];
    if (C_OUT) {
      float* cp = C + (long long)row * p.ldc + col;
      *reinterpret_cast<float4*>(cp) = make_float4(e[0], e[1], e[2], e[3]);
      *reinterpret_cast<float4*>(cp + 4) = make_float4(e[4], e[5], e[6], e[7]);
    }
    if (P_OUT && NP == 2) {
      f16x8 h, l;
#pragma unroll
      for (int c = 0; c < 8; ++c) {
        _Float16 a_, b_;
        split2h_dev(e[c], oscale, a_, b_);
        h[c] = a_; l[c] = b_;
        omx = fmaxf(omx, fabsf(e[c]));
      }
      __bf16* pp = Cp + (long long)row * p.ldcp + col;
      *reinterpret_cast<f16x8*>(pp) = h;
      *reinterpret_cast<f16x8*>(pp + p.pC) = l;
    } else if (P_OUT) {
      bf16x8 h, m, l;
#pragma unroll
      for (int c = 0; c < 8; ++c) {
        __bf16 a_, b_, c_;
        split3_dev(e[c], a_, b_, c_);
        h[c] = a_; m[c] = b_; l[c] = c_;
      }
      __bf16* pp = Cp + (long long)row * p.ldcp + col;
      *reinterpret_cast<bf16x8*>(pp) = h;
      if (NP == 3) {
        *reinterpret_cast<bf16x8*>(pp + p.pC) = m;
        *reinterpret_cast<bf16x8*>(pp + 2 * p.pC) = l;
      }
    }
    }
    }
  }
  if constexpr (NP == 2 && P_OUT) {
    const float m = block_max_val(omx, mscr);
    const int slot = FIN ? tile_id : (int)blockIdx.x;
    if (t == 0 && slot < PLANE_REC_PARTS) p.rc->amax[slot] = m;
  }
  if (p.dbp) {
    float* red = img + 2 * EG * 16 * TS;
#pragma unroll
    for (int c = 0; c < 8; ++c) csum[c] += __shfl_xor(csum[c], 32);
    if (lane < 32) {
#pragma unroll
      for (int c = 0; c < 8; ++c) red[wave * BN + oc + c] = csum[c];
    }
    __syncthreads();
    if (wave == 0 && lane < 32 && colok) {
      float t[8];
#pragma unroll
      for (int c = 0; c < 8; ++c) {
        float a = red[oc + c];
#pragma unroll
        for (int w = 1; w < WV; ++w) a += red[w * BN + oc + c];
        t[c] = a;
      }
      float* d = p.dbp + ((long long)z * nx + bx) * p.N + col;
      *reinterpret_cast<float4*>(d) = make_float4(t[0], t[1], t[2], t[3]);
      *reinterpret_cast<float4*>(d + 4) = make_float4(t[4], t[5], t[6], t[7]);
    }
  }
}

}
}
```

### mtrl_amd/csrc/heads.hip

```cpp
#include "devrng.h"
#include <algorithm>

#include <cstdlib>

#include "gemm_common.h"
#include "kernels.h"

namespace mtsac {

namespace {

constexpr float LOG2F = 0.69314718055994530942f;
constexpr float HALF_LOG_2PI = 0.91893853320467274178f;

__device__ inline float wsum(float v) {
#pragma unroll
  for (int o = 32; o > 0; o >>= 1) v += __shfl_xor(v, o);
  return v;
}

__device__ inline float softplusf(float z) {
  return fmaxf(z, 0.f) + log1pf(expf(-fabsf(z)));
}

// ... 102 lines not shown
    mu += bmu;
    ls += bls;
    float eps;
    if (p.eps != nullptr) {
      eps = eps_in;
    } else {
      float nz[4];
      const uint32_t nrow = p.noise_div > 0 ? (uint32_t)(b / p.noise_div) : (uint32_t)b;
      normal4(p.seed, p.stream_id + 16u * (uint32_t)(lane >> 2), *p.counter, nrow, nz);
      eps = nz[lane & 3];
    }
    const float lsc = fminf(fmaxf(ls, p.ls_min), p.ls_max);
    const float sigma = expf(lsc);
    const float x = mu + sigma * eps;
    const float a = tanhf(x);
    term = -0.5f * eps * eps - HALF_LOG_2PI - logf(sigma) - 2.0f * (LOG2F - x - softplusf(-2.0f * x));
    p.a_out[(long long)b * p.ld_a_out + lane] = a;
    if (p.a_out2) p.a_out2[(long long)b * p.ld_a_out2 + lane] = a;
    if (p.a_planes && p.ap_rec) {
      _Float16 h, l;
      split2h_dev(a, exp2i(p.ap_rec->e), h, l);
      const long long o = (long long)b * p.ap_ld + lane;
      reinterpret_cast<_Float16*>(p.a_planes)[o] = h;
      reinterpret_cast<_Float16*>(p.a_planes)[o + p.ap_ps] = l;
    } else if (p.a_planes) {
      __bf16 h, m, l;
      split3_dev(a, h, m, l);
      const long long o = (long long)b * p.ap_ld + lane;
      p.a_planes[o] = h;
      p.a_planes[o + p.ap_ps] = m;
      p.a_planes[o + 2 * p.ap_ps] = l;
    }
    if (p.cache) {
      float* c = p.cache + (long long)b * 5 * A;
      c[lane] = mu;
      c[A + lane] = ls;
      c[2 * A + lane] = x;
      c[3 * A + lane] = a;
      c[4 * A + lane] = eps;
    }
  }
  term = wsum(term);
  if (lane == 0) p.logpi[b] = term;
}

template <int HD>
__global__ __launch_bounds__(256) void policy_head_kernel(PolicyParams p) {
  const int lane = threadIdx.x & 63;
  const int b = blockIdx.x * 4 + (threadIdx.x >> 6);
  const HeadParams& hp = p.head;
  if (b >= hp.B) return;
  const int t = hp.task[b];
  float acc[HD];
  {
    const float* const hr[1] = {hp.h + (long long)b * hp.W};
    float a[1][HD];
    rows_dot<HD, 1>(hr, hp.Wh + (long long)t * hp.W * HD, hp.W, a,
                    hp.WhT ? hp.WhT + (long long)t * hp.W * HD : nullptr);
#pragma unroll
    for (int o = 0; o < HD; ++o) acc[o] = a[0][o];
  }
  policy_finish<HD>(p, b, t, acc, lane);
}

template <int HD, int RW>
__device__ inline void policy_head_grouped_body(const PolicyParams& p) {
  constexpr int ROWS = 4 * RW;
  const HeadParams& hp = p.head;
  const int t = blockIdx.x;
  const int n = p.counts[t];
  const int j0 = blockIdx.y * ROWS;
  if (j0 >= n) return;
  const int wave = threadIdx.x >> 6, lane = threadIdx.x & 63;
  const int* rl = p.rows + (long long)t * p.max_rows;
  int row[RW];
  const float* hr[RW];
#pragma unroll
  for (int r = 0; r < RW; ++r) {
    const int jj = j0 + wave * RW + r;
    row[r] = rl[jj < n ? jj : j0];
    hr[r] = hp.h + (long long)row[r] * hp.W;
  }
  float acc[RW][HD];
  rows_dot<HD, RW>(hr, hp.Wh + (long long)t * hp.W * HD, hp.W, acc,
                   hp.WhT ? hp.WhT + (long long)t * hp.W * HD : nullptr);
#pragma unroll
  for (int r = 0; r < RW; ++r)
    if (j0 + wave * RW + r < n) policy_finish<HD>(p, row[r], t, acc[r], lane);
}

template <int HD, int RW>
__global__ __launch_bounds__(256) void policy_head_grouped_kernel(PolicyParams p) {
  policy_head_grouped_body<HD, RW>(p);
}

template <int HD, int RW>
__global__ __launch_bounds__(256) void policy_head_pair_kernel(PolicyPair pp) {
  policy_head_grouped_body<HD, RW>(pp.p[blockIdx.z]);
}

static int rows_per_wave(long long wgs_at_rw1) {
  static const int forced = [] {
    const char* e = getenv("MTSAC_HEAD_RW");
    const int v = e ? atoi(e) : 0;
    return v == 1 || v == 2 || v == 4 ? v : 0;
  }();
  if (forced) return forced;
  for (int rw = 4; rw > 1; rw >>= 1)
    if (wgs_at_rw1 / rw >= 1024) return rw;
  return 1;
}

__global__ __launch_bounds__(256) void critic_head_kernel(CriticHeadParams p) {
  const int lane = threadIdx.x & 63;
  const HeadParams& hp = p.head;
  const int wid = blockIdx.x * 4 + (threadIdx.x >> 6);
  float dqmax = 0.f;
  for (int b = wid; b < hp.B; b += gridDim.x * 4) {
  const int t = hp.task[b];
  float q[4];
  const int E = hp.E;
  for (int e = 0; e < E; ++e) {
    float acc[1];
    head_dot<1>(hp.h + e * hp.sh + (long long)b * hp.W, hp.Wh + e * hp.sWh + (long long)t * hp.W, hp.W, acc);
    q[e] = acc[0] + hp.bh[e * hp.sbh + t];
  }
  float qt[4];
  if (p.fused_target) {
    const HeadParams& th = p.thead;
    for (int e = 0; e < E; ++e) {
      float acc[1];
      head_dot<1>(th.h + e * th.sh + (long long)b * th.W, th.Wh + e * th.sWh + (long long)t * th.W, th.W, acc);
      qt[e] = acc[0] + th.bh[e * th.sbh + t];
    }
  }
  if (lane != 0) continue;
  const float alpha = expf(p.log_alpha[p.task_begin + t]);
  float w = 1.f;
  if (p.tw != nullptr) w = p.tw[b];
  auto td_target = [&](const float* qq) {
    float mn = qq[0];
    for (int e = 1; e < E; ++e) mn = fminf(mn, qq[e]);
    const float mnext = mn - alpha * p.logpi[b];
    float y = p.rew[b] + (1.0f - p.done[b]) * p.gamma * mnext;
    if (p.clip) y = fminf(fmaxf(y, -5000.f), 5000.f);
    p.y_out[b] = y;
    return y;
  };
  if (p.mode == CH_TARGET) {
    td_target(q);
  } else if (p.mode == CH_CRITIC) {
    const float y = p.fused_target ? td_target(qt) : p.y[b];
    float sq = 0.f, qs = 0.f;
    for (int e = 0; e < E; ++e) {
      float qc = q[e], dcl = 1.f;
      if (p.clip) {
        dcl = clip_grad(qc, -5000.f, 5000.f);
        qc = fminf(fmaxf(qc, -5000.f), 5000.f);
      }
      const float diff = qc - y;
      sq += w * diff * diff;
      qs += qc;
      const float g = w * 2.0f * diff * p.inv_norm * dcl;
      p.dq[e * hp.B + b] = g;
      dqmax = fmaxf(dqmax, fabsf(g));
    }
    p.row_a[b] = sq;
    p.row_b[b] = qs;
  } else {
    float mn = q[0];
    for (int e = 1; e < E; ++e) mn = fminf(mn, q[e]);
    int cnt = 0;
    for (int e = 0; e < E; ++e) cnt += (q[e] == mn) ? 1 : 0;
    for (int e = 0; e < E; ++e) {
      const float g = (q[e] == mn) ? (-w * p.inv_norm / (float)cnt) : 0.f;
      p.dq[e * hp.B + b] = g;
      dqmax = fmaxf(dqmax, fabsf(g));
    }
    p.row_a[b] = w * (alpha * p.logpi[b] - mn);
    p.alpha_w[b] = w * alpha * p.inv_norm;
  }
  }
  if (p.dq_rec) {
    __shared__ float smx[4];
    if (lane == 0) smx[threadIdx.x >> 6] = dqmax;
    __syncthreads();
    if (threadIdx.x == 0) p.dq_rec->amax[blockIdx.x] = fmaxf(fmaxf(smx[0], smx[1]), fmaxf(smx[2], smx[3]));
  }
}

constexpr int HB_RS = 4;

template <int HD>
__device__ inline float4 head_bwd_val(const HeadParams& hp, const float* __restrict__ dout, long long s_dout, int e,
                                      int b, int w, const float (&wt)[4][HD]) {
  const float* d = dout + e * s_dout + (long long)b * HD;
  float g[4];
#pragma unroll
  for (int k = 0; k < 4; ++k) {
    float s = 0.f;
#pragma unroll
    for (int o = 0; o < HD; ++o) s += d[o] * wt[k][o];
    g[k] = s;
  }
  const float4 h = *reinterpret_cast<const float4*>(hp.h + e * hp.sh + (long long)b * hp.W + w);
  float4 out;
  out.x = h.x > 0.f ? g[0] : 0.f;
  out.y = h.y > 0.f ? g[1] : 0.f;
  out.z = h.z > 0.f ? g[2] : 0.f;
  out.w = h.w > 0.f ? g[3] : 0.f;
  return out;
}

template <int HD>
__device__ inline void head_bwd_put(const HeadParams& hp, int e, int b, int w, float4 out, float* __restrict__ dz,
                                    const PlaneOut& po) {
  const long long off = e * hp.sh + (long long)b * hp.W + w;
  if (dz) *reinterpret_cast<float4*>(dz + off) = out;
  if (po.p && po.rc) {
    const float v[4] = {out.x, out.y, out.z, out.w};
    f16x4 ph, pl;
#pragma unroll
    for (int k = 0; k < 4; ++k) {
      _Float16 a, b2;
      split2h_dev(v[k], po.w_add, a, b2);
      ph[k] = a;
      pl[k] = b2;
    }
    __bf16* q = po.p + e * po.sm + (long long)b * po.ld + w;
    *reinterpret_cast<f16x4*>(q) = ph;
    *reinterpret_cast<f16x4*>(q + po.ps) = pl;
  } else if (po.p) {
    typedef __bf16 bf16x4 __attribute__((ext_vector_type(4)));
    const float v[4] = {out.x, out.y, out.z, out.w};
    bf16x4 ph, pm, pl;
#pragma unroll
    for (int k = 0; k < 4; ++k) {
      const __bf16 hh = (__bf16)v[k];
      const float r1 = v[k] - (float)hh;
      const __bf16 mm = (__bf16)r1;
      ph[k] = hh;
      pm[k] = mm;
      pl[k] = (__bf16)(r1 - (float)mm);
    }
    __bf16* q = po.p + e * po.sm + (long long)b * po.ld + w;
    *reinterpret_cast<bf16x4*>(q) = ph;
    *reinterpret_cast<bf16x4*>(q + po.ps) = pm;
    *reinterpret_cast<bf16x4*>(q + 2 * po.ps) = pl;
  }
}

template <int HD>
__device__ inline float4 head_bwd_row(const HeadParams& hp, const float* __restrict__ dout, long long s_dout, int e,
                                      int b, int w, const float (&wt)[4][HD], float* __restrict__ dz,
                                      const PlaneOut& po) {
  const float4 out = head_bwd_val<HD>(hp, dout, s_dout, e, b, w, wt);
  head_bwd_put<HD>(hp, e, b, w, out, dz, po);
  return out;
}

__device__ inline unsigned digest4(unsigned d, float4 v) {
  d = __builtin_rotateleft32(d, 5) ^ __float_as_uint(v.x);
  d = __builtin_rotateleft32(d, 5) ^ __float_as_uint(v.y);
  d = __builtin_rotateleft32(d, 5) ^ __float_as_uint(v.z);
  return __builtin_rotateleft32(d, 5) ^ __float_as_uint(v.w);
}
__device__ inline void head_fault(unsigned* fault, unsigned bit) {
  if (fault) __hip_atomic_fetch_or(fault, bit, __ATOMIC_RELAXED, __HIP_MEMORY_SCOPE_AGENT);
}

template <int HD, bool COMPACT = false>
__device__ inline void head_bwd_data_body(const HeadParams& hp, const float* __restrict__ dout, long long s_dout,
                                          float* __restrict__ dz, const PlaneOut& po_in, float* __restrict__ dbp,
                                          const int* __restrict__ counts, const int* __restrict__ rows, int max_rows,
                                          int bx, int by, int bz, int gy, float4 (*red)[64], unsigned (*chk)[64],
                                          const int* __restrict__ slot = nullptr) {
  PlaneOut po = po_in;
  if (po.p && po.rc) {
    const float md = rec_max(po.rd, po.nd, reinterpret_cast<float*>(red));
    const int ec = plane_exp(po.kmul * md * (po.rw->amax[1] + po.w_add));
    po.w_add = exp2i(ec);
    if (bx == 0 && by == 0 && bz == 0 && threadIdx.x == 0) po.rc->e = ec;
  }
  const int e = bz, t = by / HB_RS, rs = by - t * HB_RS;
  const int lane = threadIdx.x & 63, rl = threadIdx.x >> 6;
  const int w = bx * 256 + 4 * lane;
  const bool ok = w < hp.W;
  const int n = counts[t];
  const int* rw = rows + (long long)t * max_rows;
// ... 574 lines not shown
                                                        int use_tw, float* __restrict__ alpha_row,
                                                        float* __restrict__ tw_row) {
  const int b = blockIdx.x * blockDim.x + threadIdx.x;
  if (b >= B) return;
  const int tg = task_begin + task[b];
  alpha_row[b] = expf(log_alpha[tg]);
  if (use_tw) {
    float mx = -log_alpha[0];
    for (int i = 1; i < T_glob; ++i) mx = fmaxf(mx, -log_alpha[i]);
    float s = 0.f;
    for (int i = 0; i < T_glob; ++i) s += expf(-log_alpha[i] - mx);
    tw_row[b] = (expf(-log_alpha[tg] - mx) / s) * (float)T_glob;
  }
}

__global__ __launch_bounds__(256) void head_transpose_kernel(const float* __restrict__ Wh, int W, int hd,
                                                             long long n, float* __restrict__ WhT) {
  const long long i = (long long)blockIdx.x * 256 + threadIdx.x;
  if (i >= n) return;
  const long long per = (long long)W * hd;
  const long long t = i / per, r = i - t * per;
  const int o = (int)(r / W), w = (int)(r - (long long)o * W);
  WhT[i] = Wh[t * per + (long long)w * hd + o];
}

}

void head_transpose(const float* Wh, int T_l, int W, int hd, float* WhT, hipStream_t st) {
  const long long n = (long long)T_l * W * hd;
  if (n <= 0) return;
  hipLaunchKernelGGL(head_transpose_kernel, dim3((unsigned)((n + 255) / 256)), dim3(256), 0, st, Wh, W, hd, n, WhT);
}

void policy_head(const PolicyParams& p, hipStream_t st) {
  const int hd = p.head.hd;
  if (p.counts != nullptr) {
    const int rw = rows_per_wave((long long)p.T_l * ((p.max_count + 3) / 4));
    dim3 grid((unsigned)p.T_l, (unsigned)((p.max_count + 4 * rw - 1) / (4 * rw)));
#define PHG(HDV)                                                                                          \
  if (rw == 4) hipLaunchKernelGGL((policy_head_grouped_kernel<HDV, 4>), grid, dim3(256), 0, st, p);        \
  else if (rw == 2) hipLaunchKernelGGL((policy_head_grouped_kernel<HDV, 2>), grid, dim3(256), 0, st, p);   \
  else hipLaunchKernelGGL((policy_head_grouped_kernel<HDV, 1>), grid, dim3(256), 0, st, p);
    if (hd == 8) { PHG(8) }
    else if (hd == 6) { PHG(6) }
    else if (hd == 4) { PHG(4) }
    else { PHG(2) }
#undef PHG
    return;
  }
  dim3 grid((p.head.B + 3) / 4);
  if (hd == 8)
    hipLaunchKernelGGL(policy_head_kernel<8>, grid, dim3(256), 0, st, p);
  else if (hd == 6)
    hipLaunchKernelGGL(policy_head_kernel<6>, grid, dim3(256), 0, st, p);
  else if (hd == 4)
    hipLaunchKernelGGL(policy_head_kernel<4>, grid, dim3(256), 0, st, p);
  else
    hipLaunchKernelGGL(policy_head_kernel<2>, grid, dim3(256), 0, st, p);
}

void policy_head_pair(const PolicyParams& a, const PolicyParams& b, hipStream_t st) {
  if (!a.counts || !b.counts || a.head.hd != b.head.hd || a.T_l != b.T_l || a.max_count != b.max_count) {
    policy_head(a, st);
    policy_head(b, st);
    return;
  }
  const int rw = rows_per_wave(2LL * a.T_l * ((a.max_count + 3) / 4));
  const dim3 grid((unsigned)a.T_l, (unsigned)((a.max_count + 4 * rw - 1) / (4 * rw)), 2);
  PolicyPair pp{};
  pp.p[0] = a;
  pp.p[1] = b;
#define PHP(HDV)                                                                                       \
  if (rw == 4) hipLaunchKernelGGL((policy_head_pair_kernel<HDV, 4>), grid, dim3(256), 0, st, pp);       \
  else if (rw == 2) hipLaunchKernelGGL((policy_head_pair_kernel<HDV, 2>), grid, dim3(256), 0, st, pp);  \
  else hipLaunchKernelGGL((policy_head_pair_kernel<HDV, 1>), grid, dim3(256), 0, st, pp);
  if (a.head.hd == 8) { PHP(8) }
  else if (a.head.hd == 6) { PHP(6) }
  else if (a.head.hd == 4) { PHP(4) }
  else { PHP(2) }
#undef PHP
}

void critic_head(const CriticHeadParams& p, hipStream_t st) {
  const int g = std::min((p.head.B + 3) / 4, PLANE_REC_PARTS);
  if (p.dq_parts) *p.dq_parts = g;
  hipLaunchKernelGGL(critic_head_kernel, dim3(g), dim3(256), 0, st, p);
}

void active_rows(const float* dq, int E, int B, int* n, int* rows, int* slot, hipStream_t st) {
  hipLaunchKernelGGL(active_rows_kernel, dim3((unsigned)E), dim3(1024), 0, st, dq, B, n, rows, slot);
}

void head_backward_data(const HeadParams& hp, const float* dout, long long s_dout, float* dz, const int* counts,
                        const int* rows, int max_rows, int T_l, hipStream_t st, PlaneOut po, float* dbp,
                        const int* slot) {
  const dim3 grid((unsigned)((hp.W + 255) / 256), (unsigned)(T_l * HB_RS), (unsigned)hp.E);
  if (slot != nullptr) {
    hipLaunchKernelGGL(head_bwd_data_compact_kernel<1>, grid, dim3(256), 0, st, hp, dout, s_dout, po, counts, rows,
                       max_rows, slot);
    return;
  }
#define HBD_LAUNCH(HDV)                                                                                  \
  hipLaunchKernelGGL(head_bwd_data_kernel<HDV>, grid, dim3(256), 0, st, hp, dout, s_dout, dz, po, dbp, counts, \
                     rows, max_rows)
  switch (hp.hd) {
    case 1: HBD_LAUNCH(1); break;
    case 2: HBD_LAUNCH(2); break;
    case 4: HBD_LAUNCH(4); break;
    case 6: HBD_LAUNCH(6); break;
    default: HBD_LAUNCH(8); break;
  }
#undef HBD_LAUNCH
}

int head_backward_chunks(int T_l) { return T_l * HB_RS; }

bool head_backward_both(const HeadParams& hp, const float* dout, long long s_dout, float* dz, const int* counts,
                        const int* rows, int max_rows, int T_l, PlaneOut po, float* dbp, float* dWh, float* dbh,
                        hipStream_t st) {
  if (hp.W % 4 != 0) return false;
  const int gw = (hp.W + 255) / 256;
  static const bool split_req = [] {
    const char* e = getenv("MTSAC_HEAD_BWD_SPLIT");
    return e && atoi(e) != 0;
  }();
  const bool split = split_req || (long long)T_l * gw * hp.E < 256;
  const dim3 grid((unsigned)(split ? gw * T_l * HB_RS * hp.E + T_l * gw * hp.E : T_l * gw * hp.E));
#define HBB_LAUNCH(HDV)                                                                                         \
  if (split)                                                                                                    \
    hipLaunchKernelGGL(head_bwd_both_kernel<HDV>, grid, dim3(256), 0, st, hp, dout, s_dout, dz, po, dbp, counts,  \
                       rows, max_rows, T_l, dWh, dbh);                                                          \
  else                                                                                                          \
    hipLaunchKernelGGL(head_bwd_fused_kernel<HDV>, grid, dim3(256), 0, st, hp, dout, s_dout, dz, po, dbp, counts, \
                       rows, max_rows, T_l, dWh, dbh)
  switch (hp.hd) {
    case 1: HBB_LAUNCH(1); break;
    case 2: HBB_LAUNCH(2); break;
    case 4: HBB_LAUNCH(4); break;
    case 6: HBB_LAUNCH(6); break;
    default: HBB_LAUNCH(8); break;
  }
#undef HBB_LAUNCH
  return true;
}

void head_backward_weight(const HeadParams& hp, const float* dout, long long s_dout, const int* counts,
                          const int* rows, int max_rows, float* dWh, float* dbh, hipStream_t st) {
  const unsigned T_l = (unsigned)(hp.sbh / hp.hd);
#define HBW_LAUNCH(K, HDV, WPB)                                                                             \
  hipLaunchKernelGGL(K<HDV>, dim3(T_l, (hp.W + WPB - 1) / WPB, hp.E), dim3(256), 0, st, hp, dout, s_dout, counts, \
                     rows, max_rows, dWh, dbh)
  const bool vec = hp.W % 4 == 0;
  switch (hp.hd) {
    case 1: if (vec) HBW_LAUNCH(head_bwd_weight_kernel, 1, 256); else HBW_LAUNCH(head_bwd_weight_scalar_kernel, 1, 64); break;
    case 2: if (vec) HBW_LAUNCH(head_bwd_weight_kernel, 2, 256); else HBW_LAUNCH(head_bwd_weight_scalar_kernel, 2, 64); break;
    case 4: if (vec) HBW_LAUNCH(head_bwd_weight_kernel, 4, 256); else HBW_LAUNCH(head_bwd_weight_scalar_kernel, 4, 64); break;
    case 6: if (vec) HBW_LAUNCH(head_bwd_weight_kernel, 6, 256); else HBW_LAUNCH(head_bwd_weight_scalar_kernel, 6, 64); break;
    default: if (vec) HBW_LAUNCH(head_bwd_weight_kernel, 8, 256); else HBW_LAUNCH(head_bwd_weight_scalar_kernel, 8, 64); break;
  }
#undef HBW_LAUNCH
}

void head_backward_weight_inject(const HeadParams& hp, const float* dout, long long s_dout, const int* counts,
                                 const int* rows, int max_rows, int T_l, float* dWh, float* dbh, hipStream_t st) {
  if (hp.hd != 8 || hp.W % 4 != 0) return;
  hipLaunchKernelGGL(head_bwd_weight_inject_kernel<8>, dim3((unsigned)T_l, (unsigned)((hp.W + 255) / 256), (unsigned)hp.E),
                     dim3(256), 0, st, hp, dout, s_dout, counts, rows, max_rows, dWh, dbh);
// ... 23 lines not shown
```

### mtrl_amd/csrc/kernels.h

```cpp
#pragma once
#include <hip/hip_runtime.h>
#include <stdint.h>

namespace mtsac {

enum GemmEpi {
  EPI_STORE = 0,
  EPI_BIAS_RELU = 1,
  EPI_RELU_MASK = 2,
};

struct GemmParams {
  const float* A;
  const float* B;
  float* C;
  const float* bias;
  const float* mask;
  float* db;
  int M, N, K;
  int lda, ldb, ldc, ldm;
  long long sA, sB, sC, sBias, sMask, sDb;
  int splits;
  int kchunk;
  float* ws;
// ... 9 lines not shown
  int S, M, N;
  float* C;
  int ldc;
  long long sC;
  const float* dbws;
  float* db;
  long long sDb;
  const float* cs_part;
  int cs_chunks;
  float* cs_db;
  long long cs_sdb;
};
void splitk_reduce(const GemmParams& p, int batch, int splits, hipStream_t st, const float* cs_part = nullptr,
                   int cs_chunks = 0, float* cs_db = nullptr, long long cs_sdb = 0);
struct DeferredFinish {
  ReduceJob j;
  int nred, ndb, ncs;
};
constexpr int FINISH_SINK_JOBS = 8;
struct FinishSink {
  DeferredFinish job[FINISH_SINK_JOBS];
  int n = 0;
};
DeferredFinish reduce_job(const GemmParams& p, int batch, int splits, const float* cs_part, int cs_chunks,
                          float* cs_db, long long cs_sdb);
DeferredFinish colsum_job(const float* part, int cols, int chunks, float* db, long long sdb);
void finish_many(FinishSink& s, int batch, hipStream_t st);
void transpose_f32(const float* in, long long s_in, float* out, long long s_out, int rows, int cols, int batch,
                   hipStream_t st);
void gemm_f32(const GemmParams& p, GemmKind kind, int epi, int batch, hipStream_t st);
void gemm_x3(const GemmParams& p, GemmKind kind, int epi, int batch, hipStream_t st);

constexpr int PLANE_REC_PARTS = 2048;
struct PlaneRec {
  int e;
  int pad[3];
  float amax[PLANE_REC_PARTS];
};

struct SplitGemmParams {
  const __bf16* A;
  long long lda, pA, sA;
  const __bf16* B;
  long long ldb, pB, sB;
  int a_kmajor, b_kmajor;
  float* C;
  int ldc;
  long long sC;
  const float* bias;
  long long sBias;
  const float* mask;
  int ldm;
  long long sMask;
  const __bf16* mask16;
  __bf16* Cp;
  long long ldcp, pC, sCp;
  int M, N, K;
  int splits, kchunk;
  float* ws;
  int dbg;
  int tag;
  int order;
  int b_frag;
  int np;
  float* dbp;
  const float* cs_part;
  int cs_chunks;
  float* cs_db;
  long long cs_sdb;
  int* cnt;
  const PlaneRec* ra;
  int na;
  const PlaneRec* rb;
  int nb;
  PlaneRec* rc;
  int bias_in_b;
  float kmul;
  long long pMask;
  int* nparts;
  FinishSink* defer;
  const int* rag_n;
  const int* rag_rows;
  int rag_ld;
};
constexpr int GEMM_X3F_CNT = 4096;
void gemm_x3p(const SplitGemmParams& p, int epi, int batch, hipStream_t st);
void splitk_finish(const SplitGemmParams& p, int epi, int S, int batch, hipStream_t st);
int gemm_x3p_splits(int M, int N, int K, int batch, bool kmajor, int np = 3);
long long gemm_x3p_ws_floats(int M, int N, int K, int batch, bool kmajor);
bool gemm_x3f_ok(const SplitGemmParams& p, int epi, int batch);
int gemm_x3f(const SplitGemmParams& p, int epi, int batch, hipStream_t st);
bool gemm_x3f_ragged_ok(const SplitGemmParams& p, int epi, int batch);
void gemm_x3f_ragged(const SplitGemmParams& p, hipStream_t st);
int gemm_x3f_tiles(int M, int N, int batch);
int gemm_x3f_row_tiles(int M);
int gemm_x3f_bm(const SplitGemmParams& p, int batch);
int gemm_x3f_max_row_tiles(int M);
int gemm_x3f_splits(int M, int N, int K, int batch);
int gemm_x3f_split_bm(int M, int N, int K, int batch);
int gemm_x3f_out_bm(const SplitGemmParams& p, int epi, int batch);
long long gemm_x3f_ws_floats(int M, int N, int K, int batch);
void gemm_x3f_ablate(const SplitGemmParams& p, int abl, int batch, hipStream_t st);
bool gemm_x3s_ok(const SplitGemmParams& p, int epi, int batch);
void gemm_x3s(const SplitGemmParams& p, int epi, int batch, hipStream_t st);
int gemm_x3s_ti(int M, int N, int batch);
void gemm_x3s_ablate(const SplitGemmParams& p, int abl, int batch, hipStream_t st);
extern int g_x3p_geo;
extern int g_x3p_dbg;
extern int g_x3_dbg;

struct SplitParams {
  const float* x;
  long long ldx, sx;
  int rows, cols;
  __bf16* out;
  long long ldo, po, so;
  int out_rows, out_cols;
  const int* e2h;
  int frag;
};
void split_planes(const SplitParams& s, bool transpose, int batch, hipStream_t st);
constexpr int COLSUM_CHUNKS = 64;
void colsum_finish(const float* part, int cols, int chunks, int batch, float* db, long long sdb, hipStream_t st);
void colsum(const float* x, int rows, int cols, int ld, long long sx, int batch, float* part, float* db,
            long long sdb, hipStream_t st);

struct PcgDev {
  unsigned long long state_hi, state_lo, inc_hi, inc_lo;
  int has_uint32;
  unsigned int uinteger;
};
void replay_indices(PcgDev* rng, const unsigned long long* jump ,
                    const long long* buf_size, int n, int* idx_out, hipStream_t st);
void replay_indices_high(PcgDev* rng, const unsigned long long* jump, long long high, int n, int* idx_out,
                         hipStream_t st);

struct GatherParams {
  const float* store;
  const int* idx;
  int n, T_l, R, obs_dim, act_dim, T_glob, task_begin;
  int ld_a, ld_c;
  float* xa;
  float* xa_next;
  float* xc;
  float* xc_next;
  float* xc_pi;
  float* rew;
  float* done;
  int* task;
  const double* rmin;
  const double* rmax;
  double norm_eps;
  int* err;
  __bf16* pa;
  long long pa_ps, pa_next;
  int pa_ld;
  __bf16 *pc, *pcn, *pcp;
  long long pc_ps;
  int pc_ld;
  PlaneRec* in_rec;
  const float* in_max;
};
void replay_gather(const GatherParams& p, hipStream_t st);
void batch_scatter(const GatherParams& p, const float* obs, const float* act, const float* nobs,
                   const float* done, const float* rew, int B, hipStream_t st);
void buffer_pack_slot(float* rec, int T_l, int R, int D, int A, const float* obs, const float* nobs,
                      const float* act, const float* rew, const float* done, hipStream_t st);
void buffer_commit_slot(const float* rec, int T_l, int R, int rcol, double* rmin, double* rmax, long long* buf_size,
                        long long size, hipStream_t st, int D = 0, float* bufmax = nullptr);
void fill_synthetic(float* store, long long cap, int T_l, int R, int obs_dim, int act_dim, int T_glob,
                    int task_begin, unsigned long long seed, hipStream_t st, float* bufmax = nullptr);
void absmax_into(const float* x, long long n, float* m, hipStream_t st);
void task_rows(const int* task, int B, int T_l, int* counts, int* rows, int max_rows, hipStream_t st);

struct HeadParams {
  const float* h;
  const float* Wh;
  const float* WhT;
  const float* bh;
  const int* task;
  int B, W, hd, E;
  long long sWh, sbh, sh;
  unsigned* fault;
};
constexpr unsigned HEAD_FAULT_WGRAD = 1u;
constexpr unsigned HEAD_FAULT_COLSUM = 2u;

struct PolicyParams {
  HeadParams head;
  const float* eps;
  unsigned long long seed;
  const unsigned long long* counter;
  unsigned int stream_id;
  int A;
  float ls_min, ls_max;
  float* a_out;
  int ld_a_out;
  float* a_out2;
  int ld_a_out2;
  __bf16* a_planes;
  long long ap_ps;
  int ap_ld;
  const PlaneRec* ap_rec;
  float* logpi;
  float* cache;
  const int* counts;
  const int* rows;
  int max_rows, T_l;
  int max_count;
  int noise_div;
};
void policy_head(const PolicyParams& p, hipStream_t st);
void head_transpose(const float* Wh, int T_l, int W, int hd, float* WhT, hipStream_t st);
struct PolicyPair {
  PolicyParams p[2];
};
void policy_head_pair(const PolicyParams& a, const PolicyParams& b, hipStream_t st);

enum CriticHeadMode { CH_TARGET = 0, CH_CRITIC = 1, CH_ACTOR = 2 };
struct CriticHeadParams {
  HeadParams head;
  int mode;
  HeadParams thead;
  int fused_target;
  const float* rew;
  const float* done;
  const float* logpi;
  const float* log_alpha;
  const int* task;
  int task_begin;
  const float* y;
  float* y_out;
  float* dq;
  float* row_a;
  float* row_b;
  const float* tw;
  float* alpha_w;
  float gamma;
  int clip;
  int use_task_weights;
  int T_glob;
  float inv_norm;
  PlaneRec* dq_rec;
  int* dq_parts;
};
void critic_head(const CriticHeadParams& p, hipStream_t st);

struct PlaneOut {
  __bf16* p;
  long long ld, ps, sm;
  PlaneRec* rc;
  const PlaneRec* rd;
  int nd;
  const PlaneRec* rw;
  float w_add, kmul;
  int* nparts;
};
void head_backward_data(const HeadParams& hp, const float* dout, long long s_dout, float* dz, const int* counts,
                        const int* rows, int max_rows, int T_l, hipStream_t st, PlaneOut po = PlaneOut{},
                        float* dbp = nullptr, const int* slot = nullptr);
void active_rows(const float* dq, int E, int B, int* n, int* rows, int* slot, hipStream_t st);
int head_backward_chunks(int T_l);
bool head_backward_both(const HeadParams& hp, const float* dout, long long s_dout, float* dz, const int* counts,
                        const int* rows, int max_rows, int T_l, PlaneOut po, float* dbp, float* dWh, float* dbh,
                        hipStream_t st);
void head_backward_weight_inject(const HeadParams& hp, const float* dout, long long s_dout, const int* counts,
// ... 196 lines not shown
```

Baseline: 229.9 SAC gradient-steps/sec.

## Fuse per-task head dot products into last trunk GEMM epilogue

The last hidden-layer GEMM epilogue now computes per-column-tile partial dot products with the task-indexed head weights and writes them to a partials buffer. Critic and policy heads sum these partials instead of rereading the full hidden activations. Final-layer activation stores can be skipped for rows that don't need them, and the backward ReLU mask can come from a byte bitmask built in the epilogue. This cuts the memory traffic of the head kernels, at the cost of extra epilogue work, weight loads, cross-lane shuffles and more complex control paths.

```diff
diff --git a/include/mtsac_debug.h b/include/mtsac_debug.h
--- a/include/mtsac_debug.h
+++ b/include/mtsac_debug.h
@@ -53,6 +53,14 @@
 int mtsac_debug_set_bfrag(int32_t mode);
 int mtsac_debug_set_actor_dense(int32_t mode);
 int mtsac_debug_actor_compact(struct mtsac_engine* engine);
+int mtsac_debug_set_head_fused(int32_t mode);
+int mtsac_debug_head_fused(struct mtsac_engine* engine);
+int mtsac_debug_gemm_x3f_head(int flags, int E, int M, int N, int K, int hd, int T, int c_rows, int wrap,
+                              const float* A, const float* W, const float* bias, const int* task, int nt,
+                              const float* Wh, float* C_plain, float* C_out, float* part, unsigned char* mask);
+int mtsac_debug_head_bwd_mask(int compact, int E, int B, int W, int T, const float* h, const float* Wh,
+                              const float* dout, const int* task, const unsigned char* active, void* out_f32,
+                              void* out_byte);
 int mtsac_debug_bfrag(struct mtsac_engine* engine);
 int mtsac_debug_force_one_stream(struct mtsac_engine* engine, int32_t on);
 int mtsac_debug_set_collective_model(struct mtsac_engine* engine, int32_t nranks, double bus_gbps, int32_t flags);
diff --git a/mtrl_amd/_lib.py b/mtrl_amd/_lib.py
--- a/mtrl_amd/_lib.py
+++ b/mtrl_amd/_lib.py
@@ -171,6 +171,10 @@
     "mtsac_debug_set_bfrag": (ctypes.c_int, [ctypes.c_int32]),
     "mtsac_debug_set_actor_dense": (ctypes.c_int, [ctypes.c_int32]),
     "mtsac_debug_actor_compact": (ctypes.c_int, [P]),
+    "mtsac_debug_set_head_fused": (ctypes.c_int, [ctypes.c_int32]),
+    "mtsac_debug_head_fused": (ctypes.c_int, [P]),
+    "mtsac_debug_head_bwd_mask": (ctypes.c_int, [ctypes.c_int] * 5 + [P] * 7),
+    "mtsac_debug_gemm_x3f_head": (ctypes.c_int, [ctypes.c_int] * 9 + [P] * 4 + [ctypes.c_int] + [P] * 5),
     "mtsac_debug_bfrag": (ctypes.c_int, [P]),
     "mtsac_debug_force_one_stream": (ctypes.c_int, [P, ctypes.c_int32]),
     "mtsac_debug_set_collective_model": (ctypes.c_int, [P, ctypes.c_int32, ctypes.c_double, ctypes.c_int32]),
diff --git a/mtrl_amd/csrc/debug.cpp b/mtrl_amd/csrc/debug.cpp
--- a/mtrl_amd/csrc/debug.cpp
+++ b/mtrl_amd/csrc/debug.cpp
@@ -540,6 +540,147 @@
   return 0;
 }
 
+int mtsac_debug_gemm_x3f_head(int flags, int E, int M, int N, int K, int hd, int T, int c_rows, int wrap,
+                              const float* A, const float* W, const float* bias, const int* task, int nt,
+                              const float* Wh, float* C_plain, float* C_out, float* part, unsigned char* mask) {
+  const bool mon = flags & 1, bfrag = (flags >> 1) & 1;
+  if (E < 1 || E > 2 || M < 1 || N < 8 || N % 8 != 0 || K < 1 || (hd != 1 && hd != 8) || T < 1 || c_rows < 0 ||
+      c_rows > M || wrap < 0 || nt < 1 || !A || !W || !bias || !task || !Wh || !C_plain || !C_out || !part || !mask ||
+      (bfrag && N % 16 != 0))
+    return -22;
+  for (int i = 0; i < nt; ++i)
+    if (task[i] < 0 || task[i] >= T) return -22;
+  const size_t nA = (size_t)E * M * K, nW = (size_t)E * N * K, nC = (size_t)E * M * N;
+  const int ny = gemm_x3f_col_tiles(N);
+  const size_t nP = (size_t)E * ny * M * hd, nM = (size_t)E * M * (N / 8);
+  Guarded gd;
+  float* dA = gd.in(A, nA);
+  float* dW = gd.in(W, nW);
+  float* dbias = gd.in(bias, (size_t)E * N);
+  int* dtask = gd.in(task, (size_t)nt);
+  float* dWh = gd.in(Wh, (size_t)E * T * hd * N);
+  auto amax = [](const float* x, size_t n) {
+    float m = 0.f;
+    for (size_t i = 0; i < n; ++i) m = std::max(m, std::fabs(x[i]));
+    return m;
+  };
+  auto pexp = [](float b) {
+    b *= 1.00390625f;
+    if (!(b > 0.f)) return 0;
+    int ex;
+    (void)std::frexp(b, &ex);
+    return 15 - ex;
+  };
+  std::vector<PlaneRec> hrec(2);
+  std::memset(hrec.data(), 0, sizeof(PlaneRec) * hrec.size());
+  const float ma = amax(A, nA), mw = amax(W, nW);
+  hrec[0].e = pexp(ma); hrec[0].amax[0] = ma;
+  hrec[1].e = pexp(mw); hrec[1].amax[0] = mw;
+  PlaneRec* rec = gd.in(hrec.data(), hrec.size());
+  const long long Kp = (K + 63) / 64 * 64;
+  __bf16* Ap = gd.mem.get<__bf16>((size_t)3 * M * Kp * E);
+  __bf16* Wp = gd.mem.get<__bf16>((size_t)3 * N * Kp * E);
+  float* dCp = gd.out<float>(nC, "plain C");
+  float* dCh = gd.out<float>(nC, "head C");
+  float* dP = gd.out<float>(nP, "partials");
+  unsigned char* dM = gd.out<unsigned char>(nM, "mask");
+  if (!gd.ok || !rec || !Ap || !Wp) return -12;
+  for (int z = 0; z < E; ++z) {
+    SplitParams sp{};
+    sp.ldx = K; sp.rows = M; sp.cols = K; sp.ldo = Kp; sp.po = (long long)M * Kp; sp.out_rows = M; sp.out_cols = (int)Kp;
+    sp.e2h = &rec[0].e;
+    sp.x = dA + (size_t)z * M * K; sp.out = Ap + (size_t)z * 3 * M * Kp;
+    split_planes(sp, false, 1, nullptr);
+    sp.x = dW + (size_t)z * N * K; sp.rows = N; sp.out = Wp + (size_t)z * 3 * N * Kp; sp.po = (long long)N * Kp;
+    sp.out_rows = N; sp.e2h = &rec[1].e; sp.frag = bfrag ? 1 : 0;
+    split_planes(sp, false, 1, nullptr);
+  }
+  SplitGemmParams g{};
+  g.np = 2;
+  g.A = Ap; g.lda = Kp; g.pA = (long long)M * Kp; g.sA = 3 * g.pA;
+  g.B = Wp; g.ldb = Kp; g.pB = (long long)N * Kp; g.sB = 3 * g.pB;
+  g.b_frag = bfrag ? 1 : 0;
+  g.bias = dbias; g.sBias = N;
+  g.M = M; g.N = N; g.K = (int)Kp;
+  g.ra = rec + 0; g.na = 1;
+  g.rb = rec + 1; g.nb = 1;
+  g.kmul = (float)K;
+  g.ldc = N; g.sC = (long long)M * N;
+  g.C = dCp;
+  gemm_x3f(g, EPI_BIAS_RELU, E, nullptr);
+  if (int rc = sync_rc("plain gemm_x3f")) return rc;
+  g.C = c_rows > 0 ? dCh : nullptr;
+  g.c_rows = c_rows;
+  g.hp_out = dP;
+  g.hp_w = dWh; g.hp_sw = (long long)T * hd * N;
+  g.hp_task = dtask; g.hp_nt = nt; g.hp_wrap = wrap; g.hp_hd = hd;
+  g.hp_mask = mon ? dM : nullptr;
+  gemm_x3f_head(g, E, nullptr);
+  if (int rc = sync_rc("gemm_x3f_head")) return rc;
+  if (int rc = gd.check()) return rc;
+  if (!gd.back(C_plain, dCp, nC) || !gd.back(C_out, dCh, nC) || !gd.back(part, dP, nP) || !gd.back(mask, dM, nM))
+    return -5;
+  return 0;
+}
+
+int mtsac_debug_head_bwd_mask(int compact, int E, int B, int W, int T, const float* h, const float* Wh,
+                              const float* dout, const int* task, const unsigned char* active, void* out_f32,
+                              void* out_byte) {
+  if (E < 1 || E > 2 || B < 1 || W < 8 || W % 8 != 0 || T < 1 || !h || !Wh || !dout || !task || !active || !out_f32 ||
+      !out_byte)
+    return -22;
+  for (int b = 0; b < B; ++b)
+    if (task[b] < 0 || task[b] >= T) return -22;
+  const size_t nh = (size_t)E * B * W;
+  std::vector<float> dq(dout, dout + (size_t)E * B);
+  if (compact)
+    for (size_t i = 0; i < dq.size(); ++i)
+      if (!active[i]) dq[i] = 0.f;
+  std::vector<unsigned char> bits(nh / 8);
+  for (size_t j = 0; j < bits.size(); ++j) {
+    unsigned m = 0;
+    for (int c = 0; c < 8; ++c) m |= h[8 * j + c] > 0.f ? 1u << c : 0u;
+    bits[j] = (unsigned char)m;
+  }
+  Guarded gd;
+  float* dh = gd.in(h, nh);
+  float* dWh = gd.in(Wh, (size_t)E * T * W);
+  float* ddq = gd.in(dq.data(), dq.size());
+  int* dtask = gd.in(task, (size_t)B);
+  unsigned char* dbits = gd.in(bits.data(), bits.size());
+  int* d_counts = gd.out<int>((size_t)T, "counts");
+  int* d_rows = gd.out<int>((size_t)T * B, "rows");
+  int* d_n = gd.out<int>(2, "n");
+  int* d_arows = gd.out<int>((size_t)E * B, "active rows");
+  int* d_slot = gd.out<int>((size_t)E * B, "slot");
+  __bf16* o1 = gd.out<__bf16>(3 * nh, "planes (fp32 mask)");
+  __bf16* o2 = gd.out<__bf16>(3 * nh, "planes (byte mask)");
+  if (!gd.ok) return -12;
+  task_rows(dtask, B, T, d_counts, d_rows, B, nullptr);
+  if (compact) active_rows(ddq, E, B, d_n, d_arows, d_slot, nullptr);
+  if (int rc = sync_rc("task_rows / active_rows")) return rc;
+  HeadParams hp{};
+  hp.h = dh;
+  hp.Wh = dWh;
+  hp.task = dtask;
+  hp.B = B; hp.W = W; hp.hd = 1; hp.E = E;
+  hp.sWh = (long long)T * W; hp.sbh = T; hp.sh = (long long)B * W;
+  PlaneOut po{};
+  po.ld = W; po.ps = (long long)B * W; po.sm = 3 * po.ps;
+  po.p = o1;
+  head_backward_data(hp, ddq, B, nullptr, d_counts, d_rows, B, T, nullptr, po, nullptr, compact ? d_slot : nullptr);
+  if (int rc = sync_rc("head_backward_data (fp32 mask)")) return rc;
+  hp.hmask = dbits;
+  hp.h = nullptr;
+  po.p = o2;
+  head_backward_data(hp, ddq, B, nullptr, d_counts, d_rows, B, T, nullptr, po, nullptr, compact ? d_slot : nullptr);
+  if (int rc = sync_rc("head_backward_data (byte mask)")) return rc;
+  if (int rc = gd.check()) return rc;
+  if (!gd.back(reinterpret_cast<__bf16*>(out_f32), o1, 3 * nh) || !gd.back(reinterpret_cast<__bf16*>(out_byte), o2, 3 * nh))
+    return -5;
+  return 0;
+}
+
 int mtsac_debug_gemm_fwd_bench(int which, int epi, int batch, int M, int N, int K, int iters, double* ms_per_launch) {
   const int outs = (epi >> 8) & 3;
   const int np = ((epi >> 10) & 1) ? 1 : 3;
diff --git a/mtrl_amd/csrc/engine.cpp b/mtrl_amd/csrc/engine.cpp
--- a/mtrl_amd/csrc/engine.cpp
+++ b/mtrl_amd/csrc/engine.cpp
@@ -21,6 +21,7 @@
 
 thread_local std::string g_last_error;
 int g_bfrag_mode = -1;
+int g_head_fused_mode = -1;
 int g_actor_dense_mode = -1;
 
 int fail(int code, const std::string& msg) {
@@ -245,6 +246,24 @@
   float* partials = nullptr;
   int *act_n = nullptr, *act_rows = nullptr, *act_slot = nullptr;
   bool actor_dense = false;
+  struct HeadReq {
+    float* out;
+    int c_rows;
+    int wrap;
+    unsigned char* mask;
+    bool used;
+  };
+  int head_fused = 1;
+  int head_fused_last = 0;
+  float *hp_c = nullptr, *hp_t = nullptr, *hp_a = nullptr, *hp_a2 = nullptr, *hp_cp = nullptr;
+  unsigned char* hmask_cp = nullptr;
+  void use_partials(HeadParams& hp, const HeadReq& r, const Net& net, int m_rows, long long row0 = 0) const {
+    if (!r.used) return;
+    hp.hp_ny = gemm_x3f_col_tiles(net.width);
+    hp.hp_sby = (long long)m_rows * net.hd;
+    hp.hp_sz = hp.hp_ny * hp.hp_sby;
+    hp.hpart = r.out + row0 * net.hd;
+  }
   int actor_compact_last = 0;
   float* ws_lane[5] = {};
   int* cnt_lane[5] = {};
@@ -549,7 +568,10 @@
       tl[tl_next].K = p.K;
       tl[tl_next].batch = batch;
     }
-    if (gemm_x3f_ok(p, epi, batch)) {
+    if (p.hp_out != nullptr) {
+      gemm_x3f_head(p, batch, cur);
+      fam_kernel[family] = std::string("gemm_x3f_kernel<208, 1, true, false, false, ") + (p.hp_hd == 8 ? "256" : "32") + ", 2>";
+    } else if (gemm_x3f_ok(p, epi, batch)) {
       const bool split = gemm_x3f(p, epi, batch, cur) > 1;
       const bool tagged = epi == EPI_BIAS_RELU && p.tag == 1 && p.Cp && !p.C;
       fam_kernel[family] = split ? std::string("gemm_x3f_kernel<") +
@@ -631,7 +653,8 @@
   }
 
   void trunk_forward(Net& net, const float* params, int which, const float* X, int ldx, float** acts, __bf16** actp,
-                     int M) {
+                     int M, HeadReq* hr = nullptr) {
+    if (hr) hr->used = false;
     const bool pl = planes && which >= 0 && actp != nullptr;
     __bf16* xp = pl ? in_planes(X) : nullptr;
     for (int i = 0; i < net.depth; ++i) {
@@ -672,6 +695,23 @@
           h2_gemm(g, i == 0 ? &r_in[inset_cur] : &ar[i - 1], &w_rec(net, which), last ? nullptr : &ar[i],
                   (float)(i == 0 ? net.in_dim : net.width), true);
         }
+        if (last && i > 0 && hr && hr->out && head_fused && h2 && !timing_serial && !snap_on) {
+          SplitGemmParams q = g;
+          q.hp_out = hr->out;
+          q.hp_hd = net.hd;
+          q.hp_w = net.hd == 1 ? params + net.off_hW : params == net.p && net.E == 1 ? net.whT : nullptr;
+          q.hp_sw = net.ms_hW;
+          q.hp_task = task;
+          q.hp_nt = B;
+          q.hp_wrap = hr->wrap;
+          q.c_rows = hr->c_rows;
+          q.hp_mask = hr->mask;
+          if (q.c_rows <= 0) q.C = nullptr;
+          if (q.hp_w != nullptr && gemm_x3f_head_ok(q, net.E)) {
+            g = q;
+            hr->used = true;
+          }
+        }
         gemmp(g, EPI_BIAS_RELU, net.E, i == 0 ? MTSAC_FAM_INPUT_FORWARD : MTSAC_FAM_FORWARD);
         continue;
       }
@@ -1405,7 +1445,12 @@
       if (cfg.use_task_weights) row_alpha(task, cfg.task_begin, log_alpha, T_g, Bl, 1, row_c, tw, cur);
     });
     const bool ol = overlap || lanes_alt;
-    const int s_cf = seg({s_in}, ol ? 2 : 1, [&] { trunk_forward(critic, critic.p, 0, xc, ld_c, hc, hcp, Bl); });
+    HeadReq rq_c{hp_c, Bl, 0, nullptr, false}, rq_t{hp_t, 0, 0, nullptr, false};
+    HeadReq rq_a{hp_a, (int)actor.krows, (int)actor.krows, nullptr, false}, rq_an{hp_a2, 0, 0, nullptr, false};
+    HeadReq rq_as{hp_a, Bl, 0, nullptr, false};
+    if (head_fused == 3) rq_a.out = rq_an.out = rq_as.out = nullptr;
+    HeadReq rq_cp{hp_cp, head_fused == 1 ? 0 : Bl, 0, head_fused == 1 ? hmask_cp : nullptr, false};
+    const int s_cf = seg({s_in}, ol ? 2 : 1, [&] { trunk_forward(critic, critic.p, 0, xc, ld_c, hc, hcp, Bl, &rq_c); });
     pf_issue = false;
     if (overlap && !p2) (void)hipStreamWaitEvent(st, ev_tail[step_par ^ 1], 0);
     const bool split_af = split_actor_req > 0 || (split_actor_req < 0 && dev_collective() && one_stream && !build &&
@@ -1413,6 +1458,7 @@
     auto pi_s = [&](PolicyParams& q) {
       q = pp;
       q.head = head(actor, actor.p, ha[actor.depth - 1], Bl, task);
+      use_partials(q.head, rq_as, actor, Bl);
       q.eps = device_noise ? nullptr : eps_c;
       q.stream_id = 2;
       q.a_out = xcp;
@@ -1423,9 +1469,10 @@
     };
     const int s_af = seg({s_in}, ol ? 0 : 2, [&] {
       if (split_af) {
-        trunk_forward(actor, actor.p, 0, xan, ld_a, han, hap_s2, Bl);
+        trunk_forward(actor, actor.p, 0, xan, ld_a, han, hap_s2, Bl, &rq_an);
         PolicyParams qn = pp;
         qn.head = head(actor, actor.p, han[actor.depth - 1], Bl, task);
+        use_partials(qn.head, rq_an, actor, Bl);
         qn.eps = device_noise ? nullptr : eps_n;
         qn.stream_id = 1;
         qn.a_out = xcn;
@@ -1435,9 +1482,10 @@
         policy_head(qn, cur);
         return;
       }
-      trunk_forward(actor, actor.p, 0, xa, ld_a, ha, hap, Ma);
+      trunk_forward(actor, actor.p, 0, xa, ld_a, ha, hap, Ma, &rq_a);
       PolicyParams q = pp;
       q.head = head(actor, actor.p, ha[actor.depth - 1], Bl, task);
+      use_partials(q.head, rq_a, actor, Ma);
       q.eps = device_noise ? nullptr : eps_c;
       q.stream_id = 2;
       q.a_out = xcp;
@@ -1447,6 +1495,7 @@
       q.cache = cache;
       PolicyParams qn = pp;
       qn.head = head(actor, actor.p, han[actor.depth - 1], Bl, task);
+      use_partials(qn.head, rq_a, actor, Ma, actor.krows);
       qn.eps = device_noise ? nullptr : eps_n;
       qn.stream_id = 1;
       qn.a_out = xcn;
@@ -1460,17 +1509,19 @@
     });
     const bool fuse_td = one_stream || timing_serial;
     const int s_tg = seg({s_af}, 0, [&] {
-      trunk_forward(critic, critic.tgt, 1, xcn, ld_c, hct, hctp, Bl);
+      trunk_forward(critic, critic.tgt, 1, xcn, ld_c, hct, hctp, Bl, &rq_t);
       if (!fuse_td) {
         CriticHeadParams c = ch;
         c.head = head(critic, critic.tgt, hct[critic.depth - 1], Bl, task);
+        use_partials(c.head, rq_t, critic, Bl);
         c.mode = CH_TARGET;
         c.logpi = logpi_n;
         c.y_out = y;
         critic_head(c, cur);
       }
     });
-    const HeadParams chp = head(critic, critic.p, hc[critic.depth - 1], Bl, task);
+    HeadParams chp = head(critic, critic.p, hc[critic.depth - 1], Bl, task);
+    use_partials(chp, rq_c, critic, Bl);
     bool c_both = false;
     const int s_cl = seg({s_cf, s_tg}, 1, [&] {
       CriticHeadParams c = ch;
@@ -1480,6 +1531,7 @@
       if (fuse_td) {
         c.fused_target = 1;
         c.thead = head(critic, critic.tgt, hct[critic.depth - 1], Bl, task);
+        use_partials(c.thead, rq_t, critic, Bl);
         c.logpi = logpi_n;
         c.y_out = y;
       }
@@ -1507,7 +1559,7 @@
     const int s_cb = backward_segs(critic, critic.p, xc, ld_c, hc, hcp, dzc, dzcp, s_cl, s_chw, Bl, [&] {
       if (split_af)
         s_afs = seg({s_in}, 1, [&] {
-          trunk_forward(actor, actor.p, 0, xa, ld_a, ha, hap, Bl);
+          trunk_forward(actor, actor.p, 0, xa, ld_a, ha, hap, Bl, &rq_as);
           PolicyParams q;
           pi_s(q);
           policy_head(q, cur);
@@ -1521,9 +1573,11 @@
       refresh_wt(critic, critic.tgt, 1, cur, true);
     });
     const int s_ap = seg({s_co, s_af, s_afs}, 1, [&] {
-      trunk_forward(critic, critic.p, 0, xcp, ld_c, hc, hcp, Bl);
+      trunk_forward(critic, critic.p, 0, xcp, ld_c, hc, hcp, Bl, &rq_cp);
       CriticHeadParams c = ch;
       c.head = head(critic, critic.p, hc[critic.depth - 1], Bl, task);
+      use_partials(c.head, rq_cp, critic, Bl);
+      if (rq_cp.used && rq_cp.mask) c.head.hmask = rq_cp.mask;
       c.mode = CH_ACTOR;
       c.logpi = logpi;
       c.dq = dq;
@@ -1537,6 +1591,8 @@
       critic_head(c, cur);
       const bool rag = actor_compact(Bl);
       actor_compact_last = rag ? 1 : 0;
+      head_fused_last = (rq_c.used ? 1 : 0) | (rq_t.used ? 2 : 0) | (rq_a.used || (rq_an.used && rq_as.used) ? 4 : 0) |
+                        (rq_cp.used ? 8 : 0) | (rq_cp.used && rq_cp.mask ? 16 : 0);
       if (rag) active_rows(dq, critic.E, Bl, act_n, act_rows, act_slot, cur);
       head_bwd(critic, c.head, dq, Bl, dzc, dzcp, false, rag ? act_slot : nullptr);
       for (int i = critic.depth - 1; i > 0; --i)
@@ -2383,8 +2439,21 @@
   if ((rc = e->alloc(&e->act_rows, (size_t)c.num_critics * B))) return bad(rc);
   if ((rc = e->alloc(&e->act_slot, (size_t)c.num_critics * B))) return bad(rc);
   {
+    const size_t nyc = (size_t)gemm_x3f_col_tiles(c.critic_width), nya = (size_t)gemm_x3f_col_tiles(c.actor_width);
+    const size_t nc = (size_t)c.num_critics * nyc * B * e->critic.hd;
+    if ((rc = e->alloc(&e->hp_c, nc))) return bad(rc);
+    if ((rc = e->alloc(&e->hp_t, nc))) return bad(rc);
+    if ((rc = e->alloc(&e->hp_cp, nc))) return bad(rc);
+    if ((rc = e->alloc(&e->hp_a, nya * e->Ma * e->actor.hd))) return bad(rc);
+    if ((rc = e->alloc(&e->hp_a2, nya * B * e->actor.hd))) return bad(rc);
+    if ((rc = e->alloc(&e->hmask_cp, (size_t)c.num_critics * B * ((c.critic_width + 7) / 8)))) return bad(rc);
+  }
+  {
     const char* v = getenv("MTSAC_ACTOR_DENSE");
     e->actor_dense = g_actor_dense_mode >= 0 ? g_actor_dense_mode != 0 : (v && atoi(v) != 0);
+    const char* hf = getenv("MTSAC_HEAD_FUSED");
+    e->head_fused = g_head_fused_mode >= 0 ? g_head_fused_mode : hf ? atoi(hf) : 1;
+    if (e->head_fused < 0 || e->head_fused > 3) e->head_fused = 1;
   }
   if ((rc = e->alloc(&e->cache, (size_t)B * 5 * e->A))) return bad(rc);
   if ((rc = e->alloc(&e->dout_a, (size_t)B * 2 * e->A))) return bad(rc);
@@ -3382,6 +3451,17 @@
   if (mode < -1 || mode > 1) return fail(-22, "actor dense mode is -1, 0 or 1");
   g_actor_dense_mode = mode;
   return 0;
+}
+
+int mtsac_debug_set_head_fused(int32_t mode) {
+  if (mode < -1 || mode > 3) return -22;
+  g_head_fused_mode = mode;
+  return 0;
+}
+
+int mtsac_debug_head_fused(mtsac_engine* h) {
+  if (!h) return -22;
+  return h->head_fused_last;
 }
 
 int mtsac_debug_actor_compact(mtsac_engine* h) {
diff --git a/mtrl_amd/csrc/gemm_x3f.hip b/mtrl_amd/csrc/gemm_x3f.hip
--- a/mtrl_amd/csrc/gemm_x3f.hip
+++ b/mtrl_amd/csrc/gemm_x3f.hip
@@ -213,6 +213,29 @@
     hipLaunchKernelGGL((gemm_x3f_kernel<BM0, EPI_RELU_MASK, false, true, true, TAG_RAGGED, 2>), grid, dim3(512), 0, st, p);
   else
     hipLaunchKernelGGL((gemm_x3f_kernel<BM0, EPI_RELU_MASK, true, false, true, TAG_RAGGED, 2>), grid, dim3(512), 0, st, p);
+}
+
+int gemm_x3f_col_tiles(int N) { return (N + x3fk::BN - 1) / x3fk::BN; }
+
+bool gemm_x3f_head_ok(const SplitGemmParams& p, int batch) {
+  return p.np == 2 && (p.hp_hd == 1 || p.hp_hd == 8) && p.hp_out != nullptr && p.hp_w != nullptr &&
+         p.hp_task != nullptr && p.hp_nt > 0 && p.Cp == nullptr && p.dbp == nullptr && p.bias != nullptr &&
+         (p.C != nullptr || p.c_rows <= 0) && p.c_rows <= p.M && p.N % 8 == 0 && p.ldc % 4 == 0 && [&] {
+           SplitGemmParams q = p;
+           if (q.C == nullptr) q.C = p.hp_out;
+           return gemm_x3f_ok(q, EPI_BIAS_RELU, batch) && x3f_slices(q, EPI_BIAS_RELU, batch) == 1;
+         }();
+}
+
+void gemm_x3f_head(const SplitGemmParams& p0, int batch, hipStream_t st) {
+  using namespace x3fk;
+  SplitGemmParams p = p0;
+  if (g_x3f_order) p.order = g_x3f_order;
+  const dim3 grid((unsigned)(((p.M + BM0 - 1) / BM0) * ((p.N + BN - 1) / BN) * batch));
+  if (p.hp_hd == 8)
+    hipLaunchKernelGGL((gemm_x3f_kernel<BM0, EPI_BIAS_RELU, true, false, false, TAG_HEAD8, 2>), grid, dim3(512), 0, st, p);
+  else
+    hipLaunchKernelGGL((gemm_x3f_kernel<BM0, EPI_BIAS_RELU, true, false, false, TAG_HEAD1, 2>), grid, dim3(512), 0, st, p);
 }
 
 int gemm_x3f(const SplitGemmParams& p0, int epi, int batch, hipStream_t st) {
diff --git a/mtrl_amd/csrc/gemm_x3f_impl.h b/mtrl_amd/csrc/gemm_x3f_impl.h
--- a/mtrl_amd/csrc/gemm_x3f_impl.h
+++ b/mtrl_amd/csrc/gemm_x3f_impl.h
@@ -20,6 +20,8 @@
 constexpr int BN = 256;
 constexpr int TAG_INPUT = 8;
 constexpr int TAG_RAGGED = 16;
+constexpr int TAG_HEAD1 = 32;
+constexpr int TAG_HEAD8 = 256;
 constexpr int KS = 64;
 
 __device__ inline bf16x8 gload_frag(const __bf16* base, unsigned voff) {
@@ -86,6 +88,9 @@
 
   constexpr bool RAG = ABL == TAG_RAGGED;
   static_assert(!RAG || (NP == 2 && !FIN && EPI == EPI_RELU_MASK && MASK16), "ragged: the split2h data grad only");
+  constexpr int HD = ABL == TAG_HEAD1 ? 1 : ABL == TAG_HEAD8 ? 8 : 0;
+  static_assert(HD == 0 || (NP == 2 && !FIN && EPI == EPI_BIAS_RELU && C_OUT && !P_OUT && WV == 8),
+                "head partials: the split2h top-layer forward only");
   const int ny = (p.N + BN - 1) / BN, nx = (p.M + BM - 1) / BM;
   int lin = blockIdx.x;
   int rag_t0 = 0, rag_n0 = 0, rag_n1 = 0;
@@ -395,6 +400,10 @@
     }
   }
   float bias[8];
+  if constexpr (HD > 0) {
+#pragma unroll
+    for (int c = 0; c < 8; ++c) bias[c] = 0.f;
+  }
   if (EPI == EPI_BIAS_RELU && colok) {
     const float4 u = *reinterpret_cast<const float4*>(p.bias + z * p.sBias + col);
     const float4 v = *reinterpret_cast<const float4*>(p.bias + z * p.sBias + col + 4);
@@ -441,11 +450,44 @@
       }
   };
   if constexpr (MPF) mask_load(0, 0);
+  constexpr int NHR = HD > 0 ? TI * RP : 1;
+  constexpr bool HPF = HD == 1;
+  int htk[NHR];
+  const float* hw0 = nullptr;
+  float4 hwb[2][HPF ? EG * RP : 1][2];
+  if constexpr (HD > 0) {
+    hw0 = p.hp_w + z * p.hp_sw + (colok ? col : 0);
+#pragma unroll
+    for (int i = 0; i < TI; ++i)
+#pragma unroll
+      for (int rp = 0; rp < RP; ++rp) {
+        int row = m0 + 16 * i + 2 * (wave + WV * rp) + (lane >> 5);
+        row = row < Mz ? row : Mz - 1;
+        if (p.hp_wrap > 0 && row >= p.hp_wrap) row -= p.hp_wrap;
+        row = row < p.hp_nt ? row : p.hp_nt - 1;
+        htk[i * RP + rp] = p.hp_task[row];
+      }
+  }
+  auto hw_load = [&](int i0, int b) {
+#pragma unroll
+    for (int g = 0; g < EG; ++g)
+#pragma unroll
+      for (int rp = 0; rp < RP; ++rp) {
+        if (i0 + g >= TI) break;
+        const float* w = hw0 + (long long)htk[(i0 + g) * RP + rp] * p.N;
+        hwb[b][g * RP + rp][0] = *reinterpret_cast<const float4*>(w);
+        hwb[b][g * RP + rp][1] = *reinterpret_cast<const float4*>(w + 4);
+      }
+  };
+  if constexpr (HPF) hw_load(0, 0);
 #pragma unroll
   for (int i0 = 0; i0 < TI; i0 += EG) {
     float* tb0 = img + ((i0 / EG) & 1) * EG * 16 * TS;
     if constexpr (MPF) {
       if (i0 + EG < TI) mask_load(i0 + EG, ((i0 / EG) + 1) & 1);
+    }
+    if constexpr (HPF) {
+      if (i0 + EG < TI) hw_load(i0 + EG, ((i0 / EG) + 1) & 1);
     }
 #pragma unroll
     for (int g = 0; g < EG; ++g) {
@@ -469,7 +511,10 @@
     const float4 u = *reinterpret_cast<const float4*>(tb + orow * TS + oc);
     const float4 v = *reinterpret_cast<const float4*>(tb + orow * TS + oc + 4);
     const int row = m0 + 16 * i + orow;
-    if (row >= Mz || !colok) continue;
+    const bool live = row < Mz && colok;
+    if constexpr (HD == 0) {
+      if (!live) continue;
+    }
     if ((ABL & 128) && p.M > 0) continue;
     float e[8] = {u.x, u.y, u.z, u.w, v.x, v.y, v.z, v.w};
     if constexpr (NP == 2) {
@@ -503,6 +548,46 @@
 #pragma unroll
       for (int c = 0; c < 8; ++c) e[c] = fmaxf(e[c] + bias[c], 0.f);
     }
+    if constexpr (HD > 0) {
+      const float* hw = hw0 + (long long)htk[i * RP + rp] * HD * p.N;
+      float hs[HD];
+#pragma unroll
+      for (int o = 0; o < HD; ++o) {
+        float4 w0, w1;
+        if constexpr (HPF) {
+          w0 = hwb[(i0 / EG) & 1][g * RP + rp][0];
+          w1 = hwb[(i0 / EG) & 1][g * RP + rp][1];
+        } else {
+          w0 = *reinterpret_cast<const float4*>(hw + (long long)o * p.N);
+          w1 = *reinterpret_cast<const float4*>(hw + (long long)o * p.N + 4);
+        }
+        const float wv[8] = {w0.x, w0.y, w0.z, w0.w, w1.x, w1.y, w1.z, w1.w};
+        float s = 0.f;
+#pragma unroll
+        for (int c = 0; c < 8; ++c) s = __builtin_fmaf(e[c], wv[c], s);
+        s = live ? s : 0.f;
+#pragma unroll
+        for (int x = 16; x > 0; x >>= 1) s += __shfl_xor(s, x);
+        hs[o] = s;
+      }
+      if ((lane & 31) == 0 && row < Mz) {
+        float* ho = p.hp_out + (((long long)z * ny + by) * p.M + row) * HD;
+        if constexpr (HD == 8) {
+          *reinterpret_cast<float4*>(ho) = make_float4(hs[0], hs[1], hs[2], hs[3]);
+          *reinterpret_cast<float4*>(ho + 4) = make_float4(hs[4], hs[5], hs[6], hs[7]);
+        } else {
+#pragma unroll
+          for (int o = 0; o < HD; ++o) ho[o] = hs[o];
+        }
+      }
+      if (!live) continue;
+      if (p.hp_mask) {
+        unsigned m = 0;
+#pragma unroll
+        for (int c = 0; c < 8; ++c) m |= e[c] > 0.f ? 1u << c : 0u;
+        p.hp_mask[((long long)z * p.M + row) * (p.N >> 3) + (col >> 3)] = (unsigned char)m;
+      }
+    }
     if (EPI == EPI_RELU_MASK) {
       if (MPF) {
         const i16x8& mh = mbuf[(i0 / EG) & 1][g * RP + rp][0];
@@ -529,7 +614,7 @@
     }
 #pragma unroll
     for (int c = 0; c < 8; ++c) csum[c] += e[c];
-    if (C_OUT) {
+    if (C_OUT && (HD == 0 || row < p.c_rows)) {
       float* cp = C + (long long)row * p.ldc + col;
       *reinterpret_cast<float4*>(cp) = make_float4(e[0], e[1], e[2], e[3]);
       *reinterpret_cast<float4*>(cp + 4) = make_float4(e[4], e[5], e[6], e[7]);
diff --git a/mtrl_amd/csrc/heads.hip b/mtrl_amd/csrc/heads.hip
--- a/mtrl_amd/csrc/heads.hip
+++ b/mtrl_amd/csrc/heads.hip
@@ -208,8 +208,20 @@
     hr[r] = hp.h + (long long)row[r] * hp.W;
   }
   float acc[RW][HD];
-  rows_dot<HD, RW>(hr, hp.Wh + (long long)t * hp.W * HD, hp.W, acc,
-                   hp.WhT ? hp.WhT + (long long)t * hp.W * HD : nullptr);
+  if (hp.hpart != nullptr) {
+#pragma unroll
+    for (int r = 0; r < RW; ++r)
+#pragma unroll
+      for (int o = 0; o < HD; ++o) {
+        const float* pp = hp.hpart + (long long)row[r] * HD + o;
+        float a = pp[0];
+        for (int y = 1; y < hp.hp_ny; ++y) a += pp[y * hp.hp_sby];
+        acc[r][o] = a;
+      }
+  } else {
+    rows_dot<HD, RW>(hr, hp.Wh + (long long)t * hp.W * HD, hp.W, acc,
+                     hp.WhT ? hp.WhT + (long long)t * hp.W * HD : nullptr);
+  }
 #pragma unroll
   for (int r = 0; r < RW; ++r)
     if (j0 + wave * RW + r < n) policy_finish<HD>(p, row[r], t, acc[r], lane);
@@ -240,27 +252,31 @@
 __global__ __launch_bounds__(256) void critic_head_kernel(CriticHeadParams p) {
   const int lane = threadIdx.x & 63;
   const HeadParams& hp = p.head;
-  const int wid = blockIdx.x * 4 + (threadIdx.x >> 6);
+  const bool tpr = hp.hpart != nullptr && (!p.fused_target || p.thead.hpart != nullptr);
+  const int wid = tpr ? blockIdx.x * 256 + threadIdx.x : blockIdx.x * 4 + (threadIdx.x >> 6);
+  const int wstep = tpr ? gridDim.x * 256 : gridDim.x * 4;
   float dqmax = 0.f;
-  for (int b = wid; b < hp.B; b += gridDim.x * 4) {
+  for (int b = wid; b < hp.B; b += wstep) {
   const int t = hp.task[b];
   float q[4];
   const int E = hp.E;
-  for (int e = 0; e < E; ++e) {
+  auto head_q = [&](const HeadParams& x, int e) {
     float acc[1];
-    head_dot<1>(hp.h + e * hp.sh + (long long)b * hp.W, hp.Wh + e * hp.sWh + (long long)t * hp.W, hp.W, acc);
-    q[e] = acc[0] + hp.bh[e * hp.sbh + t];
-  }
+    if (x.hpart != nullptr) {
+      const float* pp = x.hpart + e * x.hp_sz + b;
+      acc[0] = pp[0];
+      for (int y = 1; y < x.hp_ny; ++y) acc[0] += pp[y * x.hp_sby];
+    } else {
+      head_dot<1>(x.h + e * x.sh + (long long)b * x.W, x.Wh + e * x.sWh + (long long)t * x.W, x.W, acc);
+    }
+    return acc[0] + x.bh[e * x.sbh + t];
+  };
+  for (int e = 0; e < E; ++e) q[e] = head_q(hp, e);
   float qt[4];
   if (p.fused_target) {
-    const HeadParams& th = p.thead;
-    for (int e = 0; e < E; ++e) {
-      float acc[1];
-      head_dot<1>(th.h + e * th.sh + (long long)b * th.W, th.Wh + e * th.sWh + (long long)t * th.W, th.W, acc);
-      qt[e] = acc[0] + th.bh[e * th.sbh + t];
-    }
-  }
-  if (lane != 0) continue;
+    for (int e = 0; e < E; ++e) qt[e] = head_q(p.thead, e);
+  }
+  if (!tpr && lane != 0) continue;
   const float alpha = expf(p.log_alpha[p.task_begin + t]);
   float w = 1.f;
   if (p.tw != nullptr) w = p.tw[b];
@@ -309,6 +325,10 @@
   }
   if (p.dq_rec) {
     __shared__ float smx[4];
+    if (tpr) {
+#pragma unroll
+      for (int o = 32; o > 0; o >>= 1) dqmax = fmaxf(dqmax, __shfl_xor(dqmax, o));
+    }
     if (lane == 0) smx[threadIdx.x >> 6] = dqmax;
     __syncthreads();
     if (threadIdx.x == 0) p.dq_rec->amax[blockIdx.x] = fmaxf(fmaxf(smx[0], smx[1]), fmaxf(smx[2], smx[3]));
@@ -329,8 +349,16 @@
     for (int o = 0; o < HD; ++o) s += d[o] * wt[k][o];
     g[k] = s;
   }
+  float4 out;
+  if (hp.hmask != nullptr) {
+    const unsigned m = hp.hmask[((long long)e * hp.B + b) * (hp.W >> 3) + (w >> 3)] >> (w & 4);
+    out.x = (m & 1u) ? g[0] : 0.f;
+    out.y = (m & 2u) ? g[1] : 0.f;
+    out.z = (m & 4u) ? g[2] : 0.f;
+    out.w = (m & 8u) ? g[3] : 0.f;
+    return out;
+  }
   const float4 h = *reinterpret_cast<const float4*>(hp.h + e * hp.sh + (long long)b * hp.W + w);
-  float4 out;
   out.x = h.x > 0.f ? g[0] : 0.f;
   out.y = h.y > 0.f ? g[1] : 0.f;
   out.z = h.z > 0.f ? g[2] : 0.f;
@@ -1071,7 +1099,8 @@
 }
 
 void critic_head(const CriticHeadParams& p, hipStream_t st) {
-  const int g = std::min((p.head.B + 3) / 4, PLANE_REC_PARTS);
+  const bool tpr = p.head.hpart != nullptr && (!p.fused_target || p.thead.hpart != nullptr);
+  const int g = std::min(tpr ? (p.head.B + 255) / 256 : (p.head.B + 3) / 4, PLANE_REC_PARTS);
   if (p.dq_parts) *p.dq_parts = g;
   hipLaunchKernelGGL(critic_head_kernel, dim3(g), dim3(256), 0, st, p);
 }
diff --git a/mtrl_amd/csrc/kernels.h b/mtrl_amd/csrc/kernels.h
--- a/mtrl_amd/csrc/kernels.h
+++ b/mtrl_amd/csrc/kernels.h
@@ -115,6 +115,13 @@
   const int* rag_n;
   const int* rag_rows;
   int rag_ld;
+  float* hp_out;
+  const float* hp_w;
+  long long hp_sw;
+  const int* hp_task;
+  int hp_hd, hp_nt, hp_wrap;
+  int c_rows;
+  unsigned char* hp_mask;
 };
 constexpr int GEMM_X3F_CNT = 4096;
 void gemm_x3p(const SplitGemmParams& p, int epi, int batch, hipStream_t st);
@@ -125,6 +132,9 @@
 int gemm_x3f(const SplitGemmParams& p, int epi, int batch, hipStream_t st);
 bool gemm_x3f_ragged_ok(const SplitGemmParams& p, int epi, int batch);
 void gemm_x3f_ragged(const SplitGemmParams& p, hipStream_t st);
+bool gemm_x3f_head_ok(const SplitGemmParams& p, int batch);
+void gemm_x3f_head(const SplitGemmParams& p, int batch, hipStream_t st);
+int gemm_x3f_col_tiles(int N);
 int gemm_x3f_tiles(int M, int N, int batch);
 int gemm_x3f_row_tiles(int M);
 int gemm_x3f_bm(const SplitGemmParams& p, int batch);
@@ -215,6 +225,10 @@
   int B, W, hd, E;
   long long sWh, sbh, sh;
   unsigned* fault;
+  const float* hpart;
+  int hp_ny;
+  long long hp_sby, hp_sz;
+  const unsigned char* hmask;
 };
 constexpr unsigned HEAD_FAULT_WGRAD = 1u;
 constexpr unsigned HEAD_FAULT_COLSUM = 2u;
```

Result: no change. 231.9 SAC gradient-steps/sec (median of 6 runs) (+0.9%).
